# conroi/lcpc

Measured on AMD Instinct MI355X. Metric: field-elements committed/sec (whole node), Ligero 2^26 coeffs, higher is better.
Workload: dtype u32 limbs (255-bit prime field Ft255, Montgomery form)

## Files before the change

### lcpc_amd/csrc/ctx.cpp

```cpp
#include "internal.h"
#include <chrono>

using namespace lcpc;

namespace lcpc {


const uint8_t LBL_DT[7] = "$l//DT", LBL_PR[7] = "$l//PR", LBL_PE[7] = "$l//PE", LBL_CO[7] = "$l//CO";

void ctx_ref(lcpc_ctx* c) { c->refs.fetch_add(1); }

static void ctx_free(lcpc_ctx* c) {
  (void)hipSetDevice(c->prm.device);
  comm_release(c);
  for (const NttStep& s : c->ntt) dev_free(s.pack);
  dev_free(c->d_wq_w); dev_free(c->d_rootsls); dev_free(c->d_rootslcs);
  dev_free(c->d_rootsl); dev_free(c->d_rootslc); dev_free(c->d_qpl); dev_free(c->d_roots); dev_free(c->d_r2);
  dev_free(c->ws.d_tmp); dev_free(c->ws.d_t); dev_free(c->ws.d_mid); dev_free(c->d_scratch);
  c->verify_sets.clear();
  if (c->s_verify) (void)hipStreamDestroy(c->s_verify);
  for (unsigned k = 0; k < lcpc_ctx::N_STAGE; k++) {
    if (c->h_stage[k]) (void)hipHostFree(c->h_stage[k]);
    if (c->ev_stage[k]) (void)hipEventDestroy(c->ev_stage[k]);
  }
  for (auto* v : {&c->d_pre, &c->d_post})
    for (auto& d : *v) { dev_free(d.rowptr); dev_free(d.colidx); dev_free(d.vals); dev_free(d.vals29); }
  delete c;
}
void ctx_unref(lcpc_ctx* c) {
  if (c->refs.fetch_sub(1) == 1) ctx_free(c);
}

uint64_t ntt_mid_rows(const lcpc_ctx* c, uint64_t n_rows) {
  const bool ev = c->sw_ntt_mid_max_mb >= 0;
  if (c->ntt.size() != 2 || c->ntt[0].kernel != NttStep::K1S || n_rows == 0) return 0;
  if (!ev && c->log_n > 15) return 0;
  const uint64_t max_mb = ev ? (uint64_t)c->sw_ntt_mid_max_mb : 6144;
  if (max_mb == 0) return 0;
  const uint64_t per_row = c->n_cols * 36;
  uint64_t fit = (max_mb << 20) / per_row;
  if (fit == 0) return 0;
  if (fit >= n_rows) return n_rows;
  const uint64_t batches = (n_rows + fit - 1) / fit;
  return (n_rows + batches - 1) / batches;
}

static void wmul_table(const FieldDesc& f, const uint64_t* w_mont, int N, int W, uint32_t out[96]) {
  uint64_t v[MAXL];
  h_canon(f, v, w_mont);
  memset(out, 0, 96 * 4);
  for (int j = 0; j < N; j++) {
    uint64_t m[5] = {0, 0, 0, 0, 0};
    for (int i = 0; i < f.L; i++) m[i] = v[i];
    bool big = false;
    for (int i = f.L - 1; i >= 0; i--) {
      const uint64_t h = (f.p[i] >> 1) | (i + 1 < f.L ? f.p[i + 1] << 63 : 0);
      if (v[i] != h) { big = v[i] > h; break; }
    }
    if (big) {
      unsigned __int128 br = 0;
      for (int i = 0; i < 5; i++) { const unsigned __int128 d = (unsigned __int128)m[i] - (i < f.L ? f.p[i] : 0) - (uint64_t)br; m[i] = (uint64_t)d; br = (d >> 64) & 1; }
    }
    for (int k = 0; k < N; k++) {
      const int b = W * k, wd = b / 64, sh = b % 64;
      uint64_t x = m[wd] >> sh;
      if (sh && wd + 1 < 5) x |= m[wd + 1] << (64 - sh);
      out[N * k + j] = k < N - 1 ? (uint32_t)(x & (((uint64_t)1 << W) - 1)) : (uint32_t)x;
    }
    for (int s = 0; s < W; s++) h_add(f, v, v, v);
  }
}
static int build_wq_w(lcpc_ctx* c, int N, int W) {
  const FieldDesc* f = c->f;
  uint64_t i4[MAXL];
  memcpy(i4, f->rou, 8 * f->L);
  for (unsigned i = 0; i + 2 < f->S; i++) h_mul(*f, i4, i4, i4);
  uint32_t wt[96];
  wmul_table(*f, i4, N, W, wt);
  int rc = dev_alloc(&c->err, &c->d_wq_w, sizeof wt);
  if (rc) return rc;
  HIPCHK(c, hipMemcpy(c->d_wq_w, wt, sizeof wt, hipMemcpyHostToDevice));
  return 0;
}

static std::vector<uint32_t> clamp_table(const FieldDesc& f, int N, int W, int stride) {
  std::vector<uint32_t> tab((size_t)64 * stride, 0);
  for (int i = 0; i < 64; i++) {
    const int q = i - 24;
    uint64_t mag[5] = {0, 0, 0, 0, 0};
    unsigned __int128 cy = 0;
    for (int w = 0; w < 5; w++) { cy += (unsigned __int128)(w < f.L ? f.p[w] : 0) * (uint64_t)(q < 0 ? -q : q); mag[w] = (uint64_t)cy; cy >>= 64; }
    if (q < 0) {
      unsigned __int128 c2 = 1;
      for (int w = 0; w < 5; w++) { c2 += (unsigned __int128)(~mag[w]); mag[w] = (uint64_t)c2; c2 >>= 64; }
    }
    for (int l = 0; l < N; l++) {
      const int b = W * l, w = b / 64, sh = b % 64;
      uint64_t x = mag[w] >> sh;
      if (sh && w + 1 < 5) x |= mag[w + 1] << (64 - sh);
      tab[(size_t)i * stride + l] = l + 1 < N ? (uint32_t)(x & (((uint64_t)1 << W) - 1)) : (uint32_t)x;
    }
  }
  return tab;
}
static int limb_consts(lcpc_ctx* c, std::vector<uint32_t**>* made) {
  const int N = ntt_lns_limbs(c->NL), W = ntt_lns_limb_bits(c->NL);
  const std::vector<uint32_t> tab = clamp_table(*c->f, N, W, ntt_lns_stride(c->NL));
  if (made) { made->push_back(&c->d_qpl); made->push_back(&c->d_wq_w); }
  if (int rc = dev_alloc(&c->err, &c->d_qpl, tab.size() * 4)) return rc;
  HIPCHK(c, hipMemcpy(c->d_qpl, tab.data(), tab.size() * 4, hipMemcpyHostToDevice));
  return build_wq_w(c, N, W);
}

static void plan_passes(lcpc_ctx* c) {
  const unsigned k = c->log_n;
  const int NL = c->NL;
  const int lt_small = NL >= 6 ? 10 : (NL == 4 ? 11 : 12);
  const int lt_big = NL >= 6 ? 11 : 12;
  unsigned ltj_min = 0;
  while (((size_t)NL * 4 << ltj_min) < 128) ltj_min++;
  c->ntt.clear();
  auto add = [&](unsigned t0, unsigned s, unsigned log_tj, int lt) {
    NttStep p;
    p.log_tile = lt;
    p.a.roots = c->d_roots; p.a.roots29 = c->d_rootsl; p.a.qp29 = c->d_qpl; p.a.wq_w = c->d_wq_w;
    p.a.log_n = k; p.a.t0 = t0; p.a.s = s; p.a.log_tj = log_tj;
    p.roots29c = c->d_rootslc;
    p.mont_prefix = t0 + s == k ? (k == 0 ? 1u : (s % 2 == 0 ? 4u : 2u)) : 0u;
    c->ntt.push_back(p);
  };
  if ((int)k <= lt_small) {
    add(0, k, 0, lt_small);
    return;
  }
  int LT = lt_small;
  auto n_pass = [&](int lt) { unsigned per = lt - ltj_min, rest = k - lt; return 1 + (rest + per - 1) / per; };
  if (c->L == 4 && (k == 19 || k == 20) && !c->sw_ntt_general) {
    add(0, k - 10, 20 - k, 10);
    add(k - 10, 10, 0u, 10);
    return;
  }
  if (n_pass(lt_small) > 2 && n_pass(lt_big) < n_pass(lt_small)) LT = lt_big;
  const unsigned P = n_pass(LT);
  const unsigned s_final = LT;
  unsigned rem = k - s_final, t0 = 0;
  for (unsigned i = 0; i + 1 < P; i++) {
    const unsigned left = P - 1 - i;
    const unsigned s = (rem + left - 1) / left;
    add(t0, s, (uint32_t)LT - s, LT);
    t0 += s;
    rem -= s;
  }
  add(t0, s_final, 0u, LT);
}

static uint32_t ntt_tile_group_of(uint32_t log_n, int L, uint32_t log_tj) {
  const uint32_t tiles_log = log_n - 10;
  if (tiles_log < 3) return 0;
  uint32_t run_log = log_tj;
  for (uint32_t b = 8u * (uint32_t)L; b > 1; b >>= 1) run_log++;
  uint32_t lg = run_log <= 5 ? 11 - run_log : (run_log < 10 ? 10 - run_log : 0);
  return std::min(std::min(lg, 6u), tiles_log - 3);
}

static int build_limb_plan(lcpc_ctx* c, unsigned n_pass) {
  std::vector<uint32_t**> made;
  std::vector<NttStep> plan(n_pass);
  const int rc = [&]() -> int {
    const FieldDesc* f = c->f;
    ErrText* err = &c->err;
    const unsigned k = c->log_n, s0 = k - 10 * (n_pass - 1);
    const size_t stride = (size_t)ntt_lns_stride(c->NL);
    auto alloc = [&](uint32_t** p, size_t bytes) { made.push_back(p); return dev_alloc(err, p, bytes); };
    int r;
    if (c->L != 4) {
      uint64_t rp[2 * MAXL] = {1, 0, 0, 0};
      for (int i = 0; i < ntt_lns_limbs(c->NL) * ntt_lns_limb_bits(c->NL); i++) h_add(*f, rp, rp, rp);
      h_canon(*f, rp + f->L, rp);
      const size_t n_roots = (size_t)1 << (k - 1);
      uint32_t* d_rp = nullptr;
      if ((r = dev_alloc(err, &d_rp, 16 * f->L))) return r;
      if ((r = alloc(&c->d_rootsl, n_roots * stride * 4)) || (r = alloc(&c->d_rootslc, n_roots * stride * 4))) { dev_free(d_rp); return r; }
      hipError_t he = hipMemcpy(d_rp, rp, 16 * f->L, hipMemcpyHostToDevice);
      if (he == hipSuccess) he = launch_ntt_lns_roots(c->NL, c->d_roots, n_roots, d_rp, c->d_rootsl, nullptr);
      if (he == hipSuccess) he = launch_ntt_lns_roots(c->NL, c->d_roots, n_roots, d_rp + 2 * f->L, c->d_rootslc, nullptr);
      if (he == hipSuccess) he = hipDeviceSynchronize();
      dev_free(d_rp);
      if (he != hipSuccess) return fail_hip(err, he, "ntt_lns tables");
      if ((r = limb_consts(c, &made))) return r;
    }
    if (n_pass == 3) {
      const size_t n_sub = (size_t)1 << 19;
      if ((r = alloc(&c->d_rootsls, n_sub * stride * 4)) || (r = alloc(&c->d_rootslcs, n_sub * stride * 4))) return r;
      for (int i = 0; i < 2; i++) {
        const uint32_t* tab = i ? c->d_rootslc : c->d_rootsl;
        uint32_t* sub = i ? c->d_rootslcs : c->d_rootsls;
        HIPCHK(c, launch_ntt_lns_subtable(c->NL, tab, s0, n_sub, sub, nullptr));
      }
    }
    for (unsigned i = 0; i < n_pass; i++) {
      NttStep& p = plan[i];
      const bool sub = n_pass == 3 && i > 0, last = i + 1 == n_pass;
      p.kernel = c->L == 4 ? NttStep::K1S : NttStep::K1N;
      p.first = !last;
      p.a.roots = c->d_roots; p.a.roots29 = sub ? c->d_rootsls : c->d_rootsl; p.a.qp29 = c->d_qpl; p.a.wq_w = c->d_wq_w;
      p.a.log_n = sub ? 20u : k;
      p.a.t0 = last ? p.a.log_n - 10 : 0u;
      p.a.s = i == 0 ? s0 : 10u;
      p.a.log_tj = 10 - p.a.s;
      p.a.tile_group = p.first ? ntt_tile_group_of(p.a.log_n, c->L, p.a.log_tj) : 0u;
      p.a.canon_row_mask = sub ? (1u << (k - 20)) - 1 : 0u;
      p.roots29c = sub ? c->d_rootslcs : c->d_rootslc;
      p.mont_prefix = last && c->NL == 2 ? 4u : 0u;
      p.blk0_gone = last && c->NL != 2 && plan[i - 1].a.s >= 8 ? 1u : 0u;
      const bool nf = c->L == 4 && n_pass == 2 && (c->sw_ntt_form == 1 || (c->sw_ntt_form < 0 && s0 >= 6));
      p.a.form = nf ? 1u : 0u;
      if (nf && last) p.blk0_gone = 1u;
      p.pack_info = nf ? ntt_l9s_form_pack_info(p.a.s, p.first) : ntt_lns_pack_info(c->NL, p.a.s, p.first);
      const uint32_t n_classes = p.first != nf ? 1u << (p.a.log_n - 10) : 1u;
#ifdef LCPC_TEST_HOOKS
      if (n_pass == 3 && i == 0 && c->sw_test_fail_3pass) return LCPC_ERR_NOMEM;
#endif
      if ((r = alloc(&p.pack, (size_t)n_classes * p.pack_info.class_words * 4))) return r;
      NttPassArgs pa{};
      pa.roots29 = p.a.roots29; pa.roots29c = p.roots29c; pa.log_n = p.a.log_n; pa.t0 = p.a.t0; pa.s = p.a.s; pa.log_tj = p.a.log_tj;
      if (nf) HIPCHK(c, launch_ntt_l9s_form_pack(pa, p.first, p.pack_info, n_classes, p.pack, nullptr));
      else HIPCHK(c, launch_ntt_lns_pack(c->NL, pa, p.first, p.pack_info, n_classes, p.pack, nullptr));
    }
    HIPCHK(c, hipDeviceSynchronize());
    return 0;
  }();
  if (rc == 0) {
    c->ntt = std::move(plan);
    c->comm_canon = true;
    return 0;
  }
  for (uint32_t** p : made) { dev_free(*p); *p = nullptr; }
  if (rc != LCPC_ERR_NOMEM) return rc;
  (void)hipGetLastError();
  c->err.clear();
  return 0;
}

#define ECHK(call)                                                        \
  do {                                                                    \
    hipError_t e__ = (call);                                              \
    if (e__ != hipSuccess) return fail_hip(err, e__, #call);              \
  } while (0)

int encode_rows_device(const lcpc_ctx* c, EncodeWs* ws, const EncodeJob& j, hipStream_t st, ErrText* err, uint32_t* launches) {
  uint32_t dummy = 0;
  uint32_t& nl = launches ? *launches : dummy;
  if (j.kept_t) *j.kept_t = false;
  const uint64_t n_rows = j.n_rows;
  if (n_rows == 0) return 0;
  if (c->prm.encoding == LCPC_ENC_LIGERO) {
    uint64_t rb = ws->mid_failed ? 0 : ntt_mid_rows(c, n_rows);
    if (rb) {
      ErrText scratch_err;
      uint64_t want = rb * c->n_cols * 36;
#ifdef LCPC_TEST_HOOKS
      if (c->sw_test_fail_mid) want = (uint64_t)1 << 62;
#endif
      if (ensure_dev(&scratch_err, &ws->d_mid, &ws->mid_cap, want)) {
        (void)hipGetLastError();
        ws->mid_failed = true; ws->mid_cap = 0; rb = 0;
      }
    }
    const uint64_t batch = rb ? rb : n_rows;
    for (uint64_t r0 = 0; r0 < n_rows; r0 += batch) {
      const uint64_t nr = std::min(batch, n_rows - r0), consumed = r0 * j.src_stride;
      for (size_t i = 0; i < c->ntt.size(); i++) {
        const NttStep& p = c->ntt[i];
        const bool first = i == 0;
        const uint64_t len = (uint64_t)1 << p.a.log_n;
        NttPassArgs a = p.a;
        if (j.canon_out) { a.roots29c = p.roots29c; a.mont_prefix = p.mont_prefix; a.blk0_gone = p.blk0_gone; }
        a.dst = j.dst + r0 * c->n_cols * c->NL;
        a.src = first ? j.src + consumed * c->NL : a.dst;
        a.src_stride = first ? j.src_stride : len;
        a.dst_stride = len;
        a.n_valid = first ? j.n_valid : len;
        a.n_src_total = !first || j.n_src_total == ~(uint64_t)0 ? ~(uint64_t)0 : (j.n_src_total > consumed ? j.n_src_total - consumed : 0);
        a.copy_dst = first && j.copy_dst ? j.copy_dst + consumed * c->NL : nullptr;
        a.n_rows = nr << (c->log_n - p.a.log_n);
        a.mid = rb ? ws->d_mid : nullptr;
        switch (p.kernel) {
          case NttStep::K1S: ECHK(launch_ntt_pass_l9s(a, p.first, p.pack, p.pack_info, st)); break;
          case NttStep::K1N: ECHK(launch_ntt_pass_lns(c->NL, a, p.first, p.pack, p.pack_info, st)); break;
          case NttStep::GENERAL: ECHK(launch_ntt_pass(c->NL, p.log_tile, a, st)); break;
        }
        nl++;
      }
    }
    return 0;
  }
  const size_t t = c->d_pre.size();
  const DevCsr& pl = c->d_pre[t - 1];
  const size_t eb = elem_bytes(c);
  if (int rc = ensure_dev(err, &ws->d_tmp, &ws->tmp_cap, n_rows * pl.n_out * eb)) return rc;
  if (n_rows >= SDIG_T_MIN_ROWS) {
    if (int rc = ensure_dev(err, &ws->d_t, &ws->t_cap, n_rows * c->n_cols * eb)) return rc;
    ECHK(launch_transpose_to_t(c->NL, j.src, j.src_stride, j.n_valid, n_rows, ws->d_t, st, j.n_src_total, j.copy_dst, j.canon_out && j.keep_t));
    nl++;
    SpmmTArgs a{};
    a.t = ws->d_t; a.n_rows = n_rows;
    auto mat = [&](const DevCsr& m, uint64_t in_off, uint64_t out_off, bool to_tmp) -> int {
      a.out_alt = to_tmp ? ws->d_tmp : nullptr; a.in_off = in_off; a.out_off = out_off;
      a.rowptr = m.rowptr; a.colidx = m.colidx; a.vals = m.vals; a.vals29 = m.vals29; a.m = m.n_out;
      ECHK(launch_spmm_t(c->NL, a, st));
      nl++;
      return 0;
    };
    auto rs = [&](uint64_t out_off, uint64_t n_out) -> int {
      ECHK(launch_sdig_rs_t(c->NL, ws->d_tmp, (uint32_t)pl.n_out, ws->d_t, out_off, (uint32_t)n_out, n_rows, c->d_r2, st));
      nl++;
      return 0;
    };
    if (int rc = sdig_walk(c, mat, rs)) return rc;
    if (j.keep_t) {
      if (j.kept_t) *j.kept_t = true;
      return 0;
    }
    ECHK(launch_transpose_from_t(c->NL, ws->d_t, c->n_cols, n_rows, j.dst, c->n_cols, st));
    nl++;
    return 0;
  }
  if (j.src != j.dst || j.src_stride != c->n_cols) {
    ECHK(launch_pad_rows(c->NL, j.src, j.src_stride, j.dst, c->n_cols, j.n_valid, n_rows, st));
    nl++;
  }
  SpmvArgs a{};
  a.mat = j.dst; a.stride = c->n_cols; a.n_rows = n_rows;
  auto mat = [&](const DevCsr& m, uint64_t in_off, uint64_t out_off, bool to_tmp) -> int {
    a.out_alt = to_tmp ? ws->d_tmp : nullptr; a.in_off = in_off; a.out_off = out_off;
    if (to_tmp) a.out_alt_stride = pl.n_out;
    a.rowptr = m.rowptr; a.colidx = m.colidx; a.vals = m.vals; a.vals29 = m.vals29; a.m = m.n_out;
    ECHK(launch_spmv(c->NL, a, st));
    nl++;
    return 0;
  };
  auto rs = [&](uint64_t out_off, uint64_t n_out) -> int {
    ECHK(launch_sdig_rs(c->NL, ws->d_tmp, pl.n_out, (uint32_t)pl.n_out, j.dst, c->n_cols, out_off, (uint32_t)n_out, n_rows, c->d_r2, st));
    nl++;
    return 0;
  };
  return sdig_walk(c, mat, rs);
}

}

extern "C" {

int lcpc_abi_version(void) { return LCPC_ABI_VERSION; }

const char* lcpc_strerror(int s) {
  switch (s) {
    case LCPC_OK: return "ok";
    case LCPC_ERR_TOO_BIG: return "n_cols is too large for this encoding";
    case LCPC_ERR_ENCODE: return "encoding error";
    case LCPC_ERR_COMMIT: return "inconsistent commitment fields";
    case LCPC_ERR_COLUMN_NUMBER: return "bad column number";
    case LCPC_ERR_OUTER_TENSOR: return "outer tensor: wrong size";
    case LCPC_ERR_DIMS: return "dimensions not valid for this encoding";
    case LCPC_ERR_ARG: return "invalid argument";
    case LCPC_ERR_STATE: return "no commitment in this object";
    case LCPC_ERR_HIP: return "HIP runtime error";
    case LCPC_ERR_NOMEM: return "out of memory";
    case LCPC_ERR_NO_DEVICE: return "no usable HIP device (this library has no CPU fallback)";
    case LCPC_ERR_XCHG: return "all-gather of the sharded commit / prove failed";
    case LCPC_ERR_NO_RCCL: return "librccl could not be loaded";
    case LCPC_VERR_NUM_COL_OPENS: return "wrong number of column openings in proof";
    case LCPC_VERR_COLUMN_PATH: return "column verification: merkle path failed";
    case LCPC_VERR_COLUMN_EVAL: return "column verification: eval dot product failed";
    case LCPC_VERR_COLUMN_DEGREE: return "column verification: degree test dot product failed";
    case LCPC_VERR_OUTER_TENSOR: return "outer tensor: wrong size";
    case LCPC_VERR_INNER_TENSOR: return "inner tensor: wrong size";
    case LCPC_VERR_ENCODING_DIMS: return "encoding dimension mismatch";
    case LCPC_VERR_ENCODE: return "encoding error";
    case LCPC_VERR_MALFORMED: return "malformed proof bytes";
  }
  return "unknown status";
}
const char* lcpc_last_error(const lcpc_ctx* c) { return c ? c->err.c_str() : ""; }

int lcpc_static_get_dims(const lcpc_params* p, uint64_t* nr, uint64_t* np, uint64_t* nc) {
  if (!p || !nr || !np || !nc) return LCPC_ERR_ARG;
  LCPC_TRY
  const FieldDesc* f = field_desc((int)p->field);
  if (!f || p->n_coeffs == 0) return LCPC_ERR_ARG;
  if (p->encoding == LCPC_ENC_LIGERO) {
    if (p->rho_num == 0 || p->rho_num >= p->rho_den) return LCPC_ERR_ARG;
    return ligero_get_dims(*f, p->n_coeffs, p->rho_num, p->rho_den, nr, np, nc) ? LCPC_ERR_TOO_BIG : 0;
  } else if (p->encoding == LCPC_ENC_SDIG) {
    SdigSpec s;
    const int code = p->sdig_code ? (int)p->sdig_code : 3;
    uint64_t npr;
    if (!sdig_spec(code, &s) || !sdig_n_per_row(*f, p->n_coeffs, code, &npr)) return LCPC_ERR_ARG;
    std::vector<LevelDims> pre, post;
    if (!sdig_level_dims(s, npr, (double)f->flog2(), pre, post)) return LCPC_ERR_DIMS;
    *nr = (p->n_coeffs + npr - 1) / npr; *np = npr; *nc = sdig_codeword_length(pre, post);
    return 0;
  }
  return LCPC_ERR_ARG;
  LCPC_CATCH((lcpc_ctx*)nullptr)
}

int lcpc_static_get_dims_ml(const lcpc_params* p, uint32_t n_vars, uint64_t* nr, uint64_t* np, uint64_t* nc) {
  if (!p || !nr || !np || !nc || n_vars >= 63) return LCPC_ERR_ARG;
  LCPC_TRY
  const FieldDesc* f = field_desc((int)p->field);
  if (!f) return LCPC_ERR_ARG;
  const uint64_t n = (uint64_t)1 << n_vars;
  if (p->encoding == LCPC_ENC_LIGERO) {
    lcpc_params q = *p;
    q.n_coeffs = n;
    int rc = lcpc_static_get_dims(&q, nr, np, nc);
    if (rc) return rc;
    if ((*nr & (*nr - 1)) || (*np & (*np - 1)) || *nr * *np != n) return LCPC_ERR_DIMS;
    return 0;
  } else if (p->encoding == LCPC_ENC_SDIG) {
    SdigSpec s;
    const int code = p->sdig_code ? (int)p->sdig_code : 3;
    uint64_t npr;
    if (!sdig_spec(code, &s) || !sdig_n_per_row(*f, n, code, &npr, true)) return LCPC_ERR_ARG;
    std::vector<LevelDims> pre, post;
    if (!sdig_level_dims(s, npr, (double)f->flog2(), pre, post)) return LCPC_ERR_DIMS;
    *nr = (n + npr - 1) / npr; *np = npr; *nc = sdig_codeword_length(pre, post);
    return 0;
  }
  return LCPC_ERR_ARG;
  LCPC_CATCH((lcpc_ctx*)nullptr)
}

static int ctx_build(lcpc_ctx* c, const lcpc_params* p) {
  const FieldDesc* f = c->f;
  ErrText* err = &c->err;
  int rc = 0;
  if (p->encoding == LCPC_ENC_LIGERO) {
    if (p->rho_num == 0 || p->rho_num >= p->rho_den) return LCPC_ERR_ARG;
    uint64_t nr, np_, nc;
    if (p->n_per_row && p->n_cols) { np_ = p->n_per_row; nc = p->n_cols; }
    else if ((rc = lcpc_static_get_dims(p, &nr, &np_, &nc))) return rc;
    if (!(np_ < nc) || (nc & (nc - 1)) || log2_ceil(nc) > f->S) return LCPC_ERR_DIMS;
    if (log2_ceil(nc) > 30) return LCPC_ERR_TOO_BIG;
    c->n_per_row = np_; c->n_cols = nc; c->log_n = (unsigned)log2_ceil(nc);
    {
      const unsigned log_half = c->log_n ? c->log_n - 1 : 0;
      const size_t n_roots = (size_t)1 << log_half;
      std::vector<uint64_t> pw((size_t)(log_half + 1) * f->L);
      uint64_t w[MAXL];
      memcpy(w, f->rou, 8 * f->L);
      for (unsigned i = 0; i < f->S - c->log_n; i++) h_mul(*f, w, w, w);
      for (unsigned j = 0; j <= log_half; j++) { memcpy(&pw[(size_t)j * f->L], w, 8 * f->L); h_mul(*f, w, w, w); }
      uint32_t *d_pw = nullptr, *d_one = nullptr;
      if ((rc = dev_alloc(err, &d_pw, pw.size() * 8)) || (rc = dev_alloc(err, &d_one, 8 * f->L)) ||
          (rc = dev_alloc(err, &c->d_roots, n_roots * 8 * f->L)) ||
          (f->L == 4 && (rc = dev_alloc(err, &c->d_rootsl, n_roots * 48))) ||
          (f->L == 4 && (rc = dev_alloc(err, &c->d_rootslc, n_roots * 48)))) {
        dev_free(d_pw); dev_free(d_one);
        return rc;
      }
      hipError_t he = hipMemcpy(d_pw, pw.data(), pw.size() * 8, hipMemcpyHostToDevice);
      if (he == hipSuccess) he = hipMemcpy(d_one, f->r, 8 * f->L, hipMemcpyHostToDevice);
      if (he == hipSuccess) he = launch_roots(c->NL, d_pw, log_half, d_one, c->d_roots, c->d_rootsl, c->d_rootslc, nullptr);
      if (he == hipSuccess) he = hipDeviceSynchronize();
      dev_free(d_pw); dev_free(d_one);
      if (he != hipSuccess) return fail_hip(err, he, "precomp_fft");
    }
    if (f->L == 4) {
      if ((rc = limb_consts(c, nullptr))) return rc;
      c->comm_canon = true;
    }
    if ((rc = dev_alloc(err, &c->d_r2, 8 * f->L))) return rc;
    HIPCHK(c, hipMemcpy(c->d_r2, f->r2, 8 * f->L, hipMemcpyHostToDevice));
    plan_passes(c);
    if (c->sw_ntt_general) return 0;
    const uint32_t np = (uint32_t)c->ntt.size();
    if (c->L == 4 ? ntt_l9s_supported(c->log_n, np, c->ntt[0].log_tile) : np >= 2 && ntt_lns_supported(c->NL, c->log_n)) return build_limb_plan(c, 2);
    if (c->L == 4 ? ntt_l9s3_supported(c->log_n) : np >= 2 && ntt_lns3_supported(c->NL, c->log_n)) return build_limb_plan(c, 3);
    return 0;
  }
  if (p->encoding != LCPC_ENC_SDIG) return LCPC_ERR_ARG;
  if (!sdig_spec((int)c->prm.sdig_code, &c->spec)) return LCPC_ERR_ARG;
  uint64_t npr = p->n_per_row;
  if (!(p->n_per_row && p->n_cols)) {
    if (!sdig_n_per_row(*f, p->n_coeffs, (int)c->prm.sdig_code, &npr)) return LCPC_ERR_ARG;
  }
  std::vector<CsrMatrix> pre, post;
  const bool dbg = c->sw_debug_timing;
  auto now = [] { return std::chrono::duration<double, std::milli>(std::chrono::steady_clock::now().time_since_epoch()).count(); };
  const double t_gen0 = now();
  if (!sdig_generate(*f, c->spec, npr, p->seed, pre, post, c->pre_dims, c->post_dims)) return LCPC_ERR_DIMS;
  const double t_gen1 = now();
  c->n_per_row = npr;
  c->n_cols = sdig_codeword_length(c->pre_dims, c->post_dims);
  if (p->n_per_row && p->n_cols && p->n_cols != c->n_cols) return LCPC_ERR_DIMS;
  uint32_t* d_rprime = nullptr;
  if (f->L == 2 || f->L == 3) {
    uint64_t rp[MAXL] = {1, 0, 0, 0};
    for (int i = 0; i < ntt_lns_limbs(c->NL) * ntt_lns_limb_bits(c->NL); i++) h_add(*f, rp, rp, rp);
    if ((rc = dev_alloc(err, &d_rprime, 8 * f->L))) return rc;
    HIPCHK(c, hipMemcpy(d_rprime, rp, 8 * f->L, hipMemcpyHostToDevice));
  }
  struct FreeRp { uint32_t*& p; ~FreeRp() { if (p) { (void)hipDeviceSynchronize(); dev_free(p); p = nullptr; } } } free_rp{d_rprime};
  auto upload = [&](const CsrMatrix& m, DevCsr& d) -> int {
    d.n_in = m.n_in; d.n_out = m.n_out;
    int r;
    if ((r = dev_alloc(err, &d.rowptr, m.rowptr.size() * 4))) return r;
    if ((r = dev_alloc(err, &d.colidx, m.colidx.size() * 4))) return r;
    if ((r = dev_alloc(err, &d.vals, m.vals.size() * 8))) return r;
    HIPCHK(c, hipMemcpy(d.rowptr, m.rowptr.data(), m.rowptr.size() * 4, hipMemcpyHostToDevice));
    HIPCHK(c, hipMemcpy(d.colidx, m.colidx.data(), m.colidx.size() * 4, hipMemcpyHostToDevice));
    HIPCHK(c, hipMemcpy(d.vals, m.vals.data(), m.vals.size() * 8, hipMemcpyHostToDevice));
    if (f->L == 4) {
      const size_t nnz = m.colidx.size();
      if ((r = dev_alloc(err, &d.vals29, (nnz + 1) * 48))) return r;
      HIPCHK(c, launch_to_r29(d.vals, nnz, d.vals29, nullptr));
      HIPCHK(c, hipMemsetAsync(d.vals29 + nnz * 12, 0, 48, nullptr));
    } else if ((f->L == 2 || f->L == 3) && d_rprime) {
      const size_t nnz = m.colidx.size();
      const size_t stride = (size_t)ntt_lns_stride(c->NL);
      if ((r = dev_alloc(err, &d.vals29, (nnz + 1) * stride * 4))) return r;
      HIPCHK(c, launch_ntt_lns_roots(c->NL, d.vals, nnz, d_rprime, d.vals29, nullptr));
      HIPCHK(c, hipMemsetAsync(d.vals29 + nnz * stride, 0, stride * 4, nullptr));
    }
    return 0;
  };
  c->d_pre.resize(pre.size());
  c->d_post.resize(post.size());
  for (size_t i = 0; i < pre.size() && !rc; i++) { rc = upload(pre[i], c->d_pre[i]); if (!rc) rc = upload(post[i], c->d_post[i]); }
  if (!rc) rc = dev_alloc(err, &c->d_r2, 8 * f->L);
  if (rc) return rc;
  HIPCHK(c, hipMemcpy(c->d_r2, f->r2, 8 * f->L, hipMemcpyHostToDevice));
  if (dbg) fprintf(stderr, "[SdigEncoding::new] matgen %.1f ms, convert + upload %.1f ms\n", t_gen1 - t_gen0, now() - t_gen1);
  return 0;
}

int lcpc_ctx_create(const lcpc_params* p, lcpc_ctx** out) {
  if (!p || !out) return LCPC_ERR_ARG;
  *out = nullptr;
  lcpc_ctx* c = nullptr;
  LCPC_TRY
  const FieldDesc* f = field_desc((int)p->field);
  if (!f || p->hash > LCPC_HASH_SHA256) return LCPC_ERR_ARG;
  if (p->hash != LCPC_HASH_BLAKE3 && p->shard_count > 1) return LCPC_ERR_ARG;
  int ndev = 0;
  if (hipGetDeviceCount(&ndev) != hipSuccess || ndev <= 0 || p->device < 0 || p->device >= ndev) return LCPC_ERR_NO_DEVICE;
  if (hipSetDevice(p->device) != hipSuccess) return LCPC_ERR_NO_DEVICE;
  c = new lcpc_ctx();
  c->prm = *p;
  c->f = f; c->L = f->L; c->NL = 2 * f->L;
  if (c->prm.sdig_code == 0) c->prm.sdig_code = 3;
  c->sw_ntt_general = getenv("LCPC_NTT_GENERAL") != nullptr;
  if (const char* ev = getenv("LCPC_NTT_FORM")) c->sw_ntt_form = !strcmp(ev, "dif") ? 0 : (!strcmp(ev, "coset") ? 1 : -1);
  if (const char* ev = getenv("LCPC_NTT_MID_MAX_MB")) c->sw_ntt_mid_max_mb = (int64_t)strtoull(ev, nullptr, 10);
  if (const char* ev = getenv("LCPC_HOST_STAGE")) c->sw_host_stage = (int32_t)strtol(ev, nullptr, 10);
  c->sw_debug_timing = getenv("LCPC_DEBUG_TIMING") != nullptr;
#ifdef LCPC_TEST_HOOKS
  if (const char* ev = getenv("LCPC_TEST_FAIL")) {
    c->sw_test_fail_3pass = strstr(ev, "3pass") != nullptr;
    c->sw_test_fail_mid = strstr(ev, "mid") != nullptr;
  }
#endif
  int rc = 0;
  if (c->prm.shard_count > 1 && c->prm.shard_rank >= c->prm.shard_count) rc = LCPC_ERR_ARG;
  if (!rc) rc = ctx_build(c, p);
  if (rc) { ctx_unref(c); return rc; }
  c->np2 = next_pow2(c->n_cols);
  c->path_len = (uint32_t)log2_ceil(c->n_cols);
  if (c->sw_host_stage > 0) {
    c->stage_cap = (size_t)64 << 20;
    for (unsigned k = 0; k < 2; k++) {
      if (hipHostMalloc(reinterpret_cast<void**>(&c->h_stage[k]), c->stage_cap, hipHostMallocDefault) != hipSuccess) { (void)hipGetLastError(); c->h_stage[k] = nullptr; break; }
      if (hipEventCreateWithFlags(&c->ev_stage[k], hipEventDisableTiming) != hipSuccess) { (void)hipGetLastError(); (void)hipHostFree(c->h_stage[k]); c->h_stage[k] = nullptr; c->ev_stage[k] = nullptr; break; }
    }
  }
  *out = c;
  return 0;
  } catch (...) {
    if (c) ctx_unref(c);
    return LCPC_ERR_NOMEM;
  }
}

void lcpc_ctx_destroy(lcpc_ctx* c) {
  if (c) ctx_unref(c);
}

int lcpc_get_dims(const lcpc_ctx* c, uint64_t len, uint64_t* nr, uint64_t* np, uint64_t* nc) {
  if (!c || len == 0) return LCPC_ERR_ARG;
  if (nr) *nr = (len + c->n_per_row - 1) / c->n_per_row;
  if (np) *np = c->n_per_row;
  if (nc) *nc = c->n_cols;
  return 0;
}
int lcpc_dims_ok(const lcpc_ctx* c, uint64_t n_per_row, uint64_t n_cols) {
  if (!c) return 0;
  bool ok = n_per_row < n_cols && n_per_row == c->n_per_row && n_cols == c->n_cols;
  if (c->prm.encoding == LCPC_ENC_LIGERO) ok = ok && (n_cols & (n_cols - 1)) == 0;
  return ok ? 1 : 0;
}
uint64_t lcpc_get_n_col_opens(const lcpc_ctx* c) {
  if (!c) return 0;
  return c->prm.encoding == LCPC_ENC_LIGERO ? ligero_n_col_opens(c->prm.rho_num, c->prm.rho_den) : sdig_n_col_opens((int)c->prm.sdig_code);
}
uint64_t lcpc_get_n_degree_tests(const lcpc_ctx* c) { return c ? n_degree_tests(128, c->n_cols, c->f->flog2()) : 0; }
uint32_t lcpc_field_limbs(const lcpc_ctx* c) { return c ? (uint32_t)c->L : 0; }

int lcpc_encode_rows(lcpc_ctx* c, uint64_t* rows, uint64_t n_rows) {
  if (!c || !rows) return LCPC_ERR_ARG;
  if (n_rows == 0) return 0;
  LCPC_TRY
  std::lock_guard<std::mutex> g(c->mu);
  HIPCHK(c, hipSetDevice(c->prm.device));
  const size_t bytes = (size_t)n_rows * c->n_cols * elem_bytes(c);
  int rc = ensure_dev(&c->err, &c->d_scratch, &c->scratch_cap, bytes);
  if (rc) return rc;
  HIPCHK(c, hipMemcpy(c->d_scratch, rows, bytes, hipMemcpyHostToDevice));
  EncodeJob j;
  j.src = c->d_scratch; j.src_stride = c->n_cols; j.n_valid = c->n_cols; j.dst = c->d_scratch; j.n_rows = n_rows;
  if ((rc = encode_rows_device(c, &c->ws, j, nullptr, &c->err, nullptr))) return rc;
  HIPCHK(c, hipMemcpy(rows, c->d_scratch, bytes, hipMemcpyDeviceToHost));
  return 0;
  LCPC_CATCH(c)
}

}

namespace lcpc {
int encode_msgs_host(lcpc_ctx* c, const uint64_t* const* msgs, uint64_t n_rows, uint64_t* out) {
  if (n_rows == 0) return 0;
  std::lock_guard<std::mutex> g(c->mu);
  HIPCHK(c, hipSetDevice(c->prm.device));
  if (!c->s_verify) HIPCHK(c, hipStreamCreateWithFlags(&c->s_verify, hipStreamNonBlocking));
  hipStream_t st = c->s_verify;
  struct Drain { hipStream_t st; ~Drain() { (void)hipStreamSynchronize(st); } } drain{st};
  const size_t eb = elem_bytes(c);
  const size_t in_b = ((size_t)n_rows * c->n_per_row * eb + 255) & ~(size_t)255, out_b = (size_t)n_rows * c->n_cols * eb;
  int rc = ensure_dev(&c->err, &c->d_scratch, &c->scratch_cap, in_b + out_b);
  if (rc) return rc;
  uint8_t* base = reinterpret_cast<uint8_t*>(c->d_scratch);
  for (uint64_t i = 0; i < n_rows; i++)
    HIPCHK(c, hipMemcpyAsync(base + i * c->n_per_row * eb, msgs[i], c->n_per_row * eb, hipMemcpyHostToDevice, st));
  EncodeJob j;
  j.src = reinterpret_cast<uint32_t*>(base); j.src_stride = c->n_per_row; j.n_valid = c->n_per_row;
  j.dst = reinterpret_cast<uint32_t*>(base + in_b); j.n_rows = n_rows;
  if ((rc = encode_rows_device(c, &c->ws, j, st, &c->err, nullptr))) return rc;
  HIPCHK(c, hipMemcpyAsync(out, base + in_b, out_b, hipMemcpyDeviceToHost, st));
  HIPCHK(c, hipStreamSynchronize(st));
  return 0;
}
}

extern "C" {

int lcpc_field_sum_device(lcpc_ctx* c, const uint64_t* parts, uint32_t n_parts, uint64_t n_elems, void* stream, uint64_t* out) {
  if (!c || !parts || !out || n_parts == 0) return LCPC_ERR_ARG;
  hipError_t he = hipSetDevice(c->prm.device);
  if (he == hipSuccess)
    he = launch_field_sum(c->NL, reinterpret_cast<const uint32_t*>(parts), n_parts, n_elems, reinterpret_cast<uint32_t*>(out), (hipStream_t)stream);
  if (he != hipSuccess) {
    std::lock_guard<std::mutex> g(c->mu);
    return fail_hip(&c->err, he, "lcpc_field_sum_device");
  }
  return 0;
}

void lcpc_root_bincode(const uint8_t root[32], uint8_t out[40]) {
  const uint64_t l = 32;
  memcpy(out, &l, 8);
  memcpy(out + 8, root, 32);
}
void lcpc_free(void* p) { lcpc::proof_buf_free(p); }

}
```

### lcpc_amd/csrc/field_ln.h

```cpp
#pragma once
#include "field_dev.h"

namespace lcpc {

template <int NL, int W> constexpr u32 mod_limb(int k) {
  const int b = W * k, w = b / 32, sh = b % 32;
  const u64 lo = Mod<NL>::P[w], hi = (w + 1 < NL) ? Mod<NL>::P[w + 1] : 0;
  return (u32)(((lo | (hi << 32)) >> sh) & ((1u << W) - 1));
}
template <int FID> struct LnField;
template <> struct LnField<FT63> {
  static constexpr int FID = FT63, N = 3, W = 26, NL = 2, WAVES = 8, STRIDE = 4;
  static constexpr u32 limb(int k) { return mod_limb<NL, W>(k); }
};
template <> struct LnField<FT127> {
  static constexpr int FID = FT127, N = 5, W = 29, NL = 4, WAVES = 7, STRIDE = 8;
  static constexpr u32 limb(int k) { return mod_limb<NL, W>(k); }
};
template <> struct LnField<FT191> {
  static constexpr int FID = FT191, N = 7, W = 29, NL = 6, WAVES = 5, STRIDE = 8;
  static constexpr u32 limb(int k) { return mod_limb<NL, W>(k); }
};
template <> struct LnField<FT255> {
  static constexpr int FID = FT255, N = 9, W = 29, NL = 8, WAVES = 4, STRIDE = 12;
  static constexpr u32 limb(int k) { return mod_limb<NL, W>(k); }
};

#include "field_ln_gen.h"
#include "field_r29_gen.h"
#include "field_wmul_gen.h"

template <int N> struct LN {
  u32 v[N];
};

namespace ln {
constexpr int QOFF = 24;
constexpr int QBIAS = 40;

template <class FT> LCPC_DEV LN<FT::N> from_packed(const Fe<FT::NL>& a) {
  constexpr int N = FT::N, W = FT::W, NL = FT::NL;
  LN<N> r;
#pragma unroll
  for (int k = 0; k < N; k++) {
    const int b = W * k, w = b / 32, sh = b % 32;
    u32 x;
    if (sh == 0) x = a.v[w];
    else if (w + 1 < NL) x = __builtin_amdgcn_alignbit(a.v[w + 1], a.v[w], sh);
    else x = a.v[w] >> sh;
    r.v[k] = k + 1 < N ? (x & ((1u << W) - 1)) : x;
  }
  return r;
}
template <class FT> LCPC_DEV void to_packed(u32* out, const u32* l) {
  constexpr int N = FT::N, W = FT::W, NL = FT::NL;
#pragma unroll
  for (int w = 0; w < NL; w++) {
    u32 x = 0;
#pragma unroll
    for (int k = 0; k < N; k++) {
      const int off = W * k - 32 * w;
      if (off >= 0 && off < 32) x |= l[k] << off;
      else if (off < 0 && off > -32) x |= l[k] >> (-off);
    }
    out[w] = x;
  }
}
template <int N> LCPC_DEV LN<N> load_limbs(const u32* t) {
  LN<N> r;
  if constexpr (N == 3) {
    const uint2 a = *reinterpret_cast<const uint2*>(t);
    r.v[0] = a.x; r.v[1] = a.y; r.v[2] = t[2];
  } else {
    const uint4 a = *reinterpret_cast<const uint4*>(t);
    r.v[0] = a.x; r.v[1] = a.y; r.v[2] = a.z; r.v[3] = a.w;
    if constexpr (N == 5) r.v[4] = t[4];
    else if constexpr (N == 7) { const uint2 b = *reinterpret_cast<const uint2*>(t + 4); r.v[4] = b.x; r.v[5] = b.y; r.v[6] = t[6]; }
    else { const uint4 b = *reinterpret_cast<const uint4*>(t + 4); r.v[4] = b.x; r.v[5] = b.y; r.v[6] = b.z; r.v[7] = b.w; r.v[8] = t[8]; }
  }
  return r;
}
template <int N> LCPC_DEV LN<N> add(const LN<N>& a, const LN<N>& b) {
  LN<N> r;
#pragma unroll
  for (int k = 0; k < N; k++) r.v[k] = a.v[k] + b.v[k];
  return r;
}
template <int N> LCPC_DEV LN<N> sub(const LN<N>& a, const LN<N>& b) {
  LN<N> r;
#pragma unroll
  for (int k = 0; k < N; k++) r.v[k] = a.v[k] - b.v[k];
  return r;
}
template <class FT> LCPC_DEV void normalize(LN<FT::N>& a) {
#pragma unroll
  for (int k = 0; k + 1 < FT::N; k++) {
    a.v[k + 1] += (u32)((int32_t)a.v[k] >> FT::W);
    a.v[k] &= (1u << FT::W) - 1;
  }
}
template <class FT> LCPC_DEV u32 clamp_q(u32 top) {
  constexpr u32 PTOP1 = FT::limb(FT::N - 1) + 1;
  constexpr int SH = 31 - __builtin_clz(PTOP1);
  constexpr u32 MAGIC = (u32)((((u64)1 << (32 + SH)) + PTOP1 - 1) / PTOP1);
  static_assert((u64)64 * PTOP1 * PTOP1 < ((u64)1 << (32 + SH)), "magic division range");
  const u32 n = top + (u32)(QOFF * PTOP1 - QBIAS);
  return __umulhi(n, MAGIC) >> SH;
}
template <class FT> LCPC_DEV LN<FT::N> clamp_row(const u32* nqp, u32 q) { return load_limbs<FT::N>(nqp + q * FT::STRIDE); }
template <class FT> LCPC_DEV void clamp_apply(LN<FT::N>& a, const LN<FT::N>& nt) {
  int32_t c = 0;
#pragma unroll
  for (int k = 0; k + 1 < FT::N; k++) {
    const int32_t d = (int32_t)(a.v[k] + nt.v[k] + (u32)c);
    a.v[k] = (u32)d & ((1u << FT::W) - 1);
    c = d >> FT::W;
  }
  a.v[FT::N - 1] = a.v[FT::N - 1] + nt.v[FT::N - 1] + (u32)c;
}
template <class FT> LCPC_DEV LN<FT::N> mul(const LN<FT::N>& a, const LN<FT::N>& w) {
  LN<FT::N> r;
  if constexpr (FT::FID == FT63) ln_mul1s_ft63(a.v, w.v, r.v);
  else if constexpr (FT::FID == FT127) ln_mul1s_ft127(a.v, w.v, r.v);
  else if constexpr (FT::FID == FT191) ln_mul1s_ft191(a.v, w.v, r.v);
  else r29_mul1s(a.v, w.v, r.v);
  return r;
}
template <class FT> constexpr bool has_mul_u = FT::N >= 5;
template <class FT> LCPC_DEV LN<FT::N> mul_u(const LN<FT::N>& a, const u32* wt) {
  static_assert(has_mul_u<FT>, "no shifted-multiples multiply for this field");
  LN<FT::N> r;
  if constexpr (FT::FID == FT127) wmul_u_ft127(a.v, wt, r.v);
  else if constexpr (FT::FID == FT191) wmul_u_ft191(a.v, wt, r.v);
  else {
    u32 np2[9];
#pragma unroll
    for (int j = 0; j < 9; j++) np2[j] = 0u - 2u * FT::limb(j);
    wmul_u(a.v, np2, wt, r.v);
  }
  return r;
}
template <class FT> struct LazyN {
  u64 c[2 * FT::N];
};
template <class FT> LCPC_DEV void lazy_zero(LazyN<FT>& a) {
#pragma unroll
  for (int k = 0; k < 2 * FT::N; k++) a.c[k] = 0;
}
template <class FT> LCPC_DEV void lazy_mac(LazyN<FT>& a, const LN<FT::N>& x, const LN<FT::N>& v) {
#pragma unroll
  for (int i = 0; i < FT::N; i++)
#pragma unroll
    for (int j = 0; j < FT::N; j++) a.c[i + j] += (u64)x.v[i] * v.v[j];
}
template <class FT> LCPC_DEV void lazy_normalize(LazyN<FT>& a) {
#pragma unroll
  for (int k = 0; k + 1 < 2 * FT::N; k++) {
    a.c[k + 1] += a.c[k] >> FT::W;
    a.c[k] &= (1u << FT::W) - 1;
  }
}
template <class FT> LCPC_DEV Fe<FT::NL> lazy_reduce(LazyN<FT>& a) {
  constexpr int N = FT::N, W = FT::W;
  constexpr u32 M = (1u << W) - 1;
  lazy_normalize<FT>(a);
  u32 m[N], r[N];
  u64 acc = 0;
#pragma unroll
  for (int k = 0; k < 2 * N; k++) {
    acc += a.c[k];
#pragma unroll
    for (int i = 0; i < N; i++) {
      const int j = k - i;
      if (i < k && j >= 1 && j < N) acc += (u64)m[i] * FT::limb(j);
    }
    if (k < N) {
      m[k] = (0u - (u32)acc) & M;
      acc += m[k];
      acc >>= W;
    } else {
      r[k - N] = (u32)acc & M;
      acc >>= W;
    }
  }
  u32 t[FT::NL];
  to_packed<FT>(t, r);
  return fe_reduce_once<FT::NL>(t);
}

LCPC_DEV void clamp(LN<9>& a, const u32* qp) {
  constexpr u32 M = (1u << 29) - 1;
  constexpr u32 PTOP1 = LnField<FT255>::limb(8) + 1;
  constexpr u64 MAGIC = (((u64)1 << 52) + PTOP1 - 1) / PTOP1;
  const u32 n = a.v[8] + (u32)(QOFF * PTOP1 - QBIAS);
  const u32 q = (u32)(((u64)n * MAGIC) >> 52);
  const u32* t = qp + q * 12;
  int32_t d[9];
#pragma unroll
  for (int k = 0; k < 9; k++) d[k] = (int32_t)(a.v[k] - t[k]);
#pragma unroll
  for (int k = 0; k < 8; k++) {
    d[k + 1] += d[k] >> 31;
    a.v[k] = (u32)d[k] & M;
  }
  a.v[8] = (u32)d[8];
}
LCPC_DEV Fe<8> to_packed_reduced(LN<9> a, const u32* qp) {
  clamp(a, qp);
  u32 t[8];
  to_packed<LnField<FT255>>(t, a.v);
  return fe_reduce_once<8>(t);
}
}

LCPC_DEV Fe<8> fe_mul_r29(const Fe<8>& a, const LN<9>& b) {
  const LN<9> x = ln::from_packed<LnField<FT255>>(a);
  u32 m[9], r[9];
  r29_columns(x.v, b.v, m, r);
  u32 t[8];
  ln::to_packed<LnField<FT255>>(t, r);
  return fe_reduce_once<8>(t);
}

LCPC_DEV Fe<8> fe_canon_r29(const Fe<8>& a) {
  using FT = LnField<FT255>;
  constexpr u32 M = (1u << 29) - 1;
  u32 x[9];
#pragma unroll
  for (int k = 0; k < 9; k++) {
    const int b = 29 * k - 5;
    u32 v;
    if (k == 0) v = (a.v[0] << 5);
    else {
      const int w = b / 32, sh = b % 32;
      if (sh == 0) v = a.v[w];
      else if (w + 1 < 8) v = __builtin_amdgcn_alignbit(a.v[w + 1], a.v[w], sh);
      else v = a.v[w] >> sh;
    }
    x[k] = v & M;
  }
  u32 m[9], r[9];
  u64 acc = 0;
#pragma unroll
  for (int k = 0; k < 17; k++) {
    if (k < 9) acc += x[k];
#pragma unroll
    for (int i = 0; i < 9; i++) {
      const int j = k - i;
      if (i < k && j >= 1 && j < 9) acc += (u64)m[i] * FT::limb(j);
    }
    if (k < 9) {
      m[k] = (0u - (u32)acc) & M;
      acc += m[k];
      acc >>= 29;
    } else {
      r[k - 9] = (u32)acc & M;
      acc >>= 29;
    }
  }
  r[8] = (u32)acc;
  u32 t[8];
  ln::to_packed<FT>(t, r);
  return fe_reduce_once<8>(t);
}

}
```

### lcpc_amd/csrc/gen/gen_r29_asm.py

```python
#!/usr/bin/env python3

N = 9


def block(terms, a_name, b_name):
    ins = []
    ops = []
    idx = {}

    def op(name, k):
        key = (name, k)
        if key not in idx:
            idx[key] = len(ops) + 1
            ops.append('"v"(%s[%d])' % (name, k) if name != "P" else '"s"(LnField<FT255>::limb(%d))' % k)
        return "%%%d" % idx[key]

    for i, j in terms:
        ins.append('"v_mad_u64_u32 %%0, vcc, %s, %s, %%0\\n\\t"' % (op(a_name, i), op(b_name, j)))
    return "    asm(" + "\n        ".join(ins) + '\n        : "+v"(acc) : ' + ", ".join(ops) + ' : "vcc");'


out = []
out.append("// GENERATED by lcpc_amd/csrc/gen/gen_r29_asm.py -- do not edit.  Column chains of fe_mul_r29 (see field_ln.h).")
out.append("// x: multiplicand limbs (u32[9]), b: twiddle limbs (u32[9]), m: quotient digits, r: result limbs")
out.append("LCPC_DEV void r29_columns(const u32* x, const u32* b, u32* m, u32* r) {")
out.append("  u64 acc = 0;")
for k in range(2 * N - 1):
    prod = [(i, k - i) for i in range(N) if 0 <= k - i < N]
    red = [(i, k - i) for i in range(N) if i < k and 1 <= k - i < N]
    out.append("  {  // column %d: %d products, %d reduction terms" % (k, len(prod), len(red)))
    out.append(block(prod, "x", "b"))
    if red:
        out.append(block(red, "m", "P"))
    if k < N:
        out.append("    m[%d] = (0u - (u32)acc) & 0x1fffffffu;" % k)
        out.append('    asm("v_mad_u64_u32 %%0, vcc, %%1, 1, %%0" : "+v"(acc) : "v"(m[%d]) : "vcc");   // + m_k * p_0 (= 1)' % k)
        out.append("    acc >>= 29;")
    else:
        out.append("    r[%d] = (u32)acc & 0x1fffffffu;" % (k - N))
        out.append("    acc >>= 29;")
    out.append("  }")
out.append("  r[8] = (u32)acc;")
out.append("}")


FT255_P = 0x663c799b6e4d2900fda9df04b9575969ef73c79086595f3002a4f20000000001
ACC = 126
PS = 92
acc = "v[%d:%d]" % (ACC, ACC + 1)
lo = "v%d" % ACC
R = lambda k: "%%%d" % k
X = lambda i: "%%%d" % (N + i)
B = lambda j: "%%%d" % (2 * N + j)
def mul1(signed):
    mad = "v_mad_i64_i32" if signed else "v_mad_u64_u32"
    shr = "v_ashrrev_i64" if signed else "v_lshrrev_b64"
    ins = []
    for j in range(1, N):
        pj = (FT255_P >> (29 * j)) & ((1 << 29) - 1)
        ins.append("s_mov_b32 s%d, 0x%x" % (PS + j - 1, ((-pj) & 0xffffffff) if signed else pj))
    first = True
    for k in range(2 * N - 1):
        for i in range(N):
            j = k - i
            if 0 <= j < N:
                ins.append("%s %s, vcc, %s, %s, %s" % (mad, acc, X(i), B(j), "0" if first else acc))
                first = False
        for i in range(N):
            j = k - i
            if i < k and 1 <= j < N:
                ins.append("%s %s, vcc, %s, s%d, %s" % (mad, acc, R(i), PS + j - 1, acc))
        if k < N and signed:
            ins.append("v_and_b32 %s, 0x1fffffff, %s" % (R(k), lo))
        elif k < N:
            ins.append("v_sub_u32 %s, 0, %s" % (R(k), lo))
            ins.append("v_and_b32 %s, 0x1fffffff, %s" % (R(k), R(k)))
            ins.append("v_mad_u64_u32 %s, vcc, %s, 1, %s" % (acc, R(k), acc))
        else:
            ins.append("v_and_b32 %s, 0x1fffffff, %s" % (R(k - N), lo))
        ins.append("%s %s, 29, %s" % (shr, acc, acc))
    ins.append("v_mov_b32 %s, %s" % (R(N - 1), lo))
    return ins


def emit(name, comment, ins):
    out.append("")
    out.append(comment)
    out.append("LCPC_DEV void %s(const u32* x, const u32* b, u32* r) {" % name)
    out.append("  asm(")
    for t in ins:
        out.append('      "%s\\n\\t"' % t)
    outs = ", ".join('"=&v"(r[%d])' % k for k in range(N))
    inps = ", ".join(['"v"(x[%d])' % i for i in range(N)] + ['"v"(b[%d])' % j for j in range(N)])
    clob = ", ".join(['"vcc"', '"v%d"' % ACC, '"v%d"' % (ACC + 1)] + ['"s%d"' % (PS + j) for j in range(N - 1)])
    out.append("      : %s\n      : %s\n      : %s);" % (outs, inps, clob))
    out.append("}")


out.append("")
out.append("// One-statement multiplies; they clobber v[%d:%d], s[%d:%d], vcc.  The asserts tie the literals to LnField<FT255>." % (ACC, ACC + 1, PS, PS + N - 2))
for j in range(1, N):
    out.append("static_assert(LnField<FT255>::limb(%d) == 0x%xu, \"gen_r29_asm.py modulus\");" % (j, (FT255_P >> (29 * j)) & ((1 << 29) - 1)))
emit("r29_mul1s", "// signed form (ln::mul<LnField<FT255>>): x limbs two's complement, |x_k| < 2^30, |value| < 16p; b as above.\n"
     "// r = x * b * 2^-261 in (-1.2p, 0.2p]: limbs 0..7 in [0, 2^29), top limb signed.", mul1(True))
print("\n".join(out))
```

### lcpc_amd/csrc/internal.h

```cpp
#pragma once
#include "../../include/lcpc_hip.h"
#include <hip/hip_runtime.h>
#include <stdio.h>
#include <stdlib.h>
#include <string.h>
#include <algorithm>
#include <atomic>
#include <condition_variable>
#include <memory>
#include <mutex>
#include <new>
#include <shared_mutex>
#include <string>
#include <thread>
#include <vector>
#include "encoding.h"
#include "host_crypto.h"
#include "host_field.h"
#include "host_par.h"
#include "kernels.h"

namespace lcpc {

struct DevCsr {
  uint64_t n_in = 0, n_out = 0;
  uint32_t *rowptr = nullptr, *colidx = nullptr, *vals = nullptr;
  uint32_t* vals29 = nullptr;
};
struct NttStep {
  enum Kernel { GENERAL, K1S, K1N } kernel = GENERAL;
  bool first = false;
  int log_tile = 0;
  NttPassArgs a{};
  const uint32_t* roots29c = nullptr;
  uint32_t mont_prefix = 0, blk0_gone = 0;
  uint32_t* pack = nullptr;
  NttPackInfo pack_info{};
};

struct EncodeWs {
  uint32_t* d_tmp = nullptr;
  uint64_t tmp_cap = 0;
  uint32_t* d_t = nullptr;
  uint64_t t_cap = 0;
  uint32_t* d_mid = nullptr;
  uint64_t mid_cap = 0;
  bool mid_failed = false;
};
uint64_t ntt_mid_rows(const lcpc_ctx* c, uint64_t n_rows);

constexpr uint64_t SDIG_T_MIN_ROWS = 24;

void* proof_buf_alloc(size_t n);
void proof_buf_free(void* p);

class ErrText {
 public:
  ErrText& operator=(const std::string& s) { set(s.c_str()); return *this; }
  ErrText& operator=(const char* s) { set(s); return *this; }
  void clear() { set(""); }
  const char* c_str() const { return buf_[cur_.load(std::memory_order_acquire)]; }
 private:
  void set(const char* s) {
    std::lock_guard<std::mutex> g(mu_);
    const unsigned k = (cur_.load(std::memory_order_relaxed) + 1) % 4;
    snprintf(buf_[k], sizeof buf_[k], "%s", s ? s : "");
    cur_.store(k, std::memory_order_release);
  }
  std::mutex mu_;
  std::atomic<unsigned> cur_{0};
  char buf_[4][512] = {};
};

class FillLock {
 public:
  void lock() {
    std::unique_lock<std::mutex> g(mu_);
    ++fills_waiting_;
    cv_.wait(g, [&] { return !filling_ && readers_ == 0; });
    --fills_waiting_;
    filling_ = true;
  }
  void unlock() {
    { std::lock_guard<std::mutex> g(mu_); filling_ = false; }
    cv_.notify_all();
  }
  void lock_shared() {
    std::unique_lock<std::mutex> g(mu_);
    cv_.wait(g, [&] { return !filling_ && fills_waiting_ == 0; });
    ++readers_;
  }
  void unlock_shared() {
    bool last;
    { std::lock_guard<std::mutex> g(mu_); last = --readers_ == 0; }
    if (last) cv_.notify_all();
  }
 private:
  std::mutex mu_;
  std::condition_variable cv_;
  unsigned readers_ = 0, fills_waiting_ = 0;
  bool filling_ = false;
};

struct DevScratch {
  uint32_t* d = nullptr;
  uint64_t cap = 0;
  uint32_t* t29 = nullptr;
  uint64_t t29_cap = 0;
  void release() { if (d) (void)hipFree(d); if (t29) (void)hipFree(t29); d = t29 = nullptr; cap = t29_cap = 0; }
};

struct CallSet {
  bool busy = false;
  uint8_t* h_pin = nullptr;
  uint64_t h_pin_cap = 0;
  hipStream_t st = nullptr;
  hipEvent_t ev_slice[2] = {nullptr, nullptr};
  DevScratch sc;
  int make();
  void quiesce() { (void)hipStreamSynchronize(st); }
  ~CallSet();
};
struct VerifySet {
  bool busy = false;
  uint8_t* h_pin = nullptr;
  uint64_t h_pin_cap = 0;
  int make() { return 0; }
  void quiesce() {}
  ~VerifySet() { if (h_pin) (void)hipHostFree(h_pin); }
};

template <typename S> class SetPool {
 public:
  static constexpr size_t MAX_SETS = 8;
  int take(uint64_t pin_bytes, S** out) {
    *out = nullptr;
    std::unique_lock<std::mutex> lk(mu_);
    bool reuse_only = false;
    for (;;) {
      S* pick = nullptr;
      for (auto& s : sets_) if (!s->busy && s->h_pin_cap >= pin_bytes) { pick = s.get(); break; }
      if (!pick && !reuse_only) {
        for (auto& s : sets_) if (!s->busy) { pick = s.get(); break; }
        if (!pick && sets_.size() < MAX_SETS) {
          std::unique_ptr<S> s(new S());
          if (int rc = s->make()) return rc;
          sets_.push_back(std::move(s));
          pick = sets_.back().get();
        }
      }
      if (!pick) {
        if (reuse_only && !any_holds(pin_bytes)) return LCPC_ERR_NOMEM;
        cv_.wait(lk);
        continue;
      }
      pick->busy = true;
      if (pick->h_pin_cap >= pin_bytes) { *out = pick; return 0; }
      lk.unlock();
      if (pick->h_pin) (void)hipHostFree(pick->h_pin);
      pick->h_pin = nullptr; pick->h_pin_cap = 0;
      void* hp = nullptr;
      const bool ok = hipHostMalloc(&hp, (size_t)pin_bytes, hipHostMallocDefault) == hipSuccess;
      if (!ok) (void)hipGetLastError();
      lk.lock();
      if (ok) { pick->h_pin = static_cast<uint8_t*>(hp); pick->h_pin_cap = pin_bytes; *out = pick; return 0; }
      pick->busy = false;
      if (!any_holds(pin_bytes)) return LCPC_ERR_NOMEM;
      reuse_only = true;
    }
  }
  void give(S* s) {
    { std::lock_guard<std::mutex> g(mu_); s->busy = false; }
    cv_.notify_all();
  }
  void clear() { sets_.clear(); }
 private:
  bool any_holds(uint64_t pin_bytes) const {
    for (auto& s : sets_) if (s->h_pin_cap >= pin_bytes) return true;
    return false;
  }
  std::mutex mu_;
  std::condition_variable cv_;
  std::vector<std::unique_ptr<S>> sets_;
};
template <typename S> struct SetLease {
  SetPool<S>& pool;
  S* s = nullptr;
  ~SetLease() { if (s) { s->quiesce(); pool.give(s); } }
};

struct BatchSlab {
  uint8_t* d = nullptr;
  uint64_t off_comm = 0, off_t = 0, off_coeffs = 0, off_hashes = 0, off_cvs = 0;
  uint64_t comm_stride = 0, t_stride = 0, coeffs_stride = 0, hashes_stride = 0, cvs_stride = 0;
  uint64_t tmp_stride = 0;
  uint32_t n_batch = 0;
  uint64_t n_rows = 0;
  uint32_t* h_roots = nullptr;
  uint32_t* d_roots_alias = nullptr;
  EncodeWs ws;
  uint32_t* seg(uint64_t off, uint64_t stride, uint32_t i) const { return reinterpret_cast<uint32_t*>(d + off) + (size_t)i * stride; }
  ~BatchSlab() {
    if (d) (void)hipFree(d);
    if (ws.d_tmp) (void)hipFree(ws.d_tmp);
    if (ws.d_t) (void)hipFree(ws.d_t);
    if (ws.d_mid) (void)hipFree(ws.d_mid);
    if (h_roots) (void)hipHostFree(h_roots);
  }
};

}

struct lcpc_transcript {
  lcpc::Transcript t;
  lcpc_transcript(const uint8_t* l, size_t n) : t(l, n) {}
};

struct lcpc_ctx {
  lcpc_params prm{};
  bool sw_ntt_general = false;
  int sw_ntt_form = -1;
  int64_t sw_ntt_mid_max_mb = -1;
  bool sw_debug_timing = false;
  bool sw_test_fail_3pass = false;
  bool sw_test_fail_mid = false;
  const lcpc::FieldDesc* f = nullptr;
  int L = 0, NL = 0;
  uint64_t n_per_row = 0, n_cols = 0, np2 = 0;
  uint32_t path_len = 0;
  unsigned log_n = 0;
  uint32_t* d_roots = nullptr;
  uint32_t* d_rootsl = nullptr;
  uint32_t* d_rootslc = nullptr;
  uint32_t* d_qpl = nullptr;
  uint32_t* d_rootsls = nullptr;
  uint32_t* d_rootslcs = nullptr;
  uint32_t* d_wq_w = nullptr;
  std::vector<lcpc::NttStep> ntt;
  bool comm_canon = false;
  lcpc::SdigSpec spec{};
  std::vector<lcpc::LevelDims> pre_dims, post_dims;
  std::vector<lcpc::DevCsr> d_pre, d_post;
  uint32_t* d_r2 = nullptr;
  lcpc::EncodeWs ws;
  uint32_t* d_scratch = nullptr;
  uint64_t scratch_cap = 0;
  void* comm = nullptr;
  std::mutex xchg_mu;
  hipEvent_t ev_xchg = nullptr;
  std::atomic<int> refs{1};
  lcpc::ErrText err;
  std::mutex mu;
  lcpc::SetPool<lcpc::VerifySet> verify_sets;
  hipStream_t s_verify = nullptr;
  std::mutex stage_mu;
  static constexpr unsigned N_STAGE = 4;
  uint8_t* h_stage[N_STAGE] = {nullptr, nullptr, nullptr, nullptr};
  hipEvent_t ev_stage[N_STAGE] = {nullptr, nullptr, nullptr, nullptr};
  size_t stage_cap = 0;
  unsigned stage_next = 0;
  int32_t sw_host_stage = -1;
};

struct lcpc_commit_s {
  lcpc_ctx* enc = nullptr;
  bool committed = false;
  uint64_t n_rows = 0;
  uint64_t row_begin = 0, n_rows_local = 0;
  uint64_t chunk_begin = 0, chunk_end = 0, n_chunks = 0;
  uint32_t *d_coeffs = nullptr, *d_comm = nullptr, *d_hashes = nullptr, *d_cvs = nullptr;
  const uint32_t* coeffs_view = nullptr;
  uint64_t cap_coeff_rows = 0, cap_comm_rows = 0, cap_cvs = 0;
  std::shared_ptr<lcpc::BatchSlab> slab;
  uint32_t slab_index = 0;
  uint32_t* d_chain = nullptr;
  uint64_t cap_chain = 0;
  lcpc::EncodeWs ws;
  bool comm_t = false;
  bool comm_rows_valid = false;
  uint32_t* d_node_tab = nullptr;
  uint64_t node_tab_key = 0;
  std::vector<uint32_t> node_slot_h, node_log_h;
  struct NodeTab { uint64_t key; uint32_t* d; std::vector<uint32_t> slot, lg; };
  std::vector<NodeTab> node_tabs;
  uint8_t* d_gather = nullptr;
  uint64_t gather_cap = 0;
  uint8_t *d_xsend = nullptr, *d_xrecv = nullptr;
  uint64_t xchg_cap = 0;
  lcpc::DevScratch sc;
  uint32_t* h_root = nullptr;
  uint32_t* d_root_alias = nullptr;
  bool timing = false;
  hipEvent_t ev[6] = {nullptr, nullptr, nullptr, nullptr, nullptr, nullptr};
  hipStream_t s_prove = nullptr;
  hipEvent_t ev_done = nullptr;
  hipStream_t s_xchg = nullptr;
  hipEvent_t ev_hashed = nullptr;
  bool shard_encoded = false;
  hipStream_t s_copy = nullptr, s_comp = nullptr;
  hipEvent_t ev_batch[16] = {nullptr};
  mutable lcpc::FillLock fill_mu;
  lcpc::SetPool<lcpc::CallSet> sets;
  std::mutex shard_prove_mu;
  lcpc_timings last{};
  uint32_t launches[3] = {0, 0, 0};
  lcpc::ErrText err;
  std::mutex mu;
};

namespace lcpc {

inline int fail_hip(ErrText* err, hipError_t e, const char* what) {
  if (err) *err = std::string(what) + ": " + hipGetErrorString(e);
  return e == hipErrorOutOfMemory ? LCPC_ERR_NOMEM : LCPC_ERR_HIP;
}
#define HIPCHK(c, call)                                                   \
  do {                                                                    \
    hipError_t e__ = (call);                                              \
    if (e__ != hipSuccess) return lcpc::fail_hip((c) ? &(c)->err : nullptr, e__, #call); \
  } while (0)

#define LCPC_TRY try {
#define LCPC_CATCH(c)                                                     \
  } catch (const std::bad_alloc&) {                                       \
    if (c) (c)->err = "host allocation failed";                          \
    return LCPC_ERR_NOMEM;                                                \
  } catch (const std::exception& ex__) {                                  \
    if (c) (c)->err = ex__.what();                                       \
    return LCPC_ERR_STATE;                                                \
  } catch (...) {                                                         \
    return LCPC_ERR_STATE;                                                \
  }

template <typename T> int dev_alloc(ErrText* err, T** p, size_t bytes) {
  *p = nullptr;
  if (bytes == 0) bytes = 16;
  hipError_t e = hipMalloc(reinterpret_cast<void**>(p), bytes);
  if (e != hipSuccess) return fail_hip(err, e, "hipMalloc");
  return 0;
}
inline void dev_free(void* p) { if (p) (void)hipFree(p); }
template <typename T> int ensure_dev(ErrText* err, T** p, uint64_t* cap, uint64_t bytes) {
  bytes = (bytes + 255) & ~(uint64_t)255;
  if (bytes > *cap || !*p) {
    dev_free(*p);
    *p = nullptr; *cap = 0;
    int rc = dev_alloc(err, p, (size_t)bytes);
    if (rc) return rc;
    *cap = bytes;
  }
  return 0;
}

inline size_t elem_bytes(const lcpc_ctx* c) { return (size_t)8 * c->L; }
inline bool is_sha3(const lcpc_ctx* c) { return c->prm.hash == LCPC_HASH_SHA3_256; }
inline bool is_blake2b(const lcpc_ctx* c) { return c->prm.hash == LCPC_HASH_BLAKE2B; }
inline bool is_keccak256(const lcpc_ctx* c) { return c->prm.hash == LCPC_HASH_KECCAK256; }
inline bool is_sha256(const lcpc_ctx* c) { return c->prm.hash == LCPC_HASH_SHA256; }
inline bool is_blake3(const lcpc_ctx* c) { return c->prm.hash == LCPC_HASH_BLAKE3; }
inline uint32_t digest_len(const lcpc_ctx* c) { return is_blake2b(c) ? 64u : 32u; }
inline uint32_t digest_words(const lcpc_ctx* c) { return digest_len(c) / 4; }
inline uint64_t leaf_chunks(const lcpc_ctx* c, uint64_t n_rows) { return (32 + elem_bytes(c) * n_rows + 1023) / 1024; }

extern const uint8_t LBL_DT[7], LBL_PR[7], LBL_PE[7], LBL_CO[7];


void ctx_ref(lcpc_ctx* c);
void ctx_unref(lcpc_ctx* c);
struct EncodeJob {
  const uint32_t* src = nullptr;
  uint64_t src_stride = 0, n_valid = 0;
  uint32_t* dst = nullptr;
  uint64_t n_rows = 0;
  uint64_t n_src_total = ~(uint64_t)0;
  uint32_t* copy_dst = nullptr;
  bool canon_out = false;
  bool keep_t = false;
  bool* kept_t = nullptr;
};
int encode_rows_device(const lcpc_ctx* c, EncodeWs* ws, const EncodeJob& j, hipStream_t st, ErrText* err, uint32_t* launches);

int encode_msgs_host(lcpc_ctx* c, const uint64_t* const* msgs, uint64_t n_rows, uint64_t* out);

template <class Mat, class Rs> int sdig_walk(const lcpc_ctx* c, Mat&& mat, Rs&& rs) {
  const size_t t = c->d_pre.size();
  const DevCsr& pl = c->d_pre[t - 1];
  uint64_t in_start = 0;
  for (size_t i = 0; i + 1 < t; i++) {
    if (int rc = mat(c->d_pre[i], in_start, in_start + c->d_pre[i].n_in, false)) return rc;
    in_start += c->d_pre[i].n_in;
  }
  if (int rc = mat(pl, in_start, 0, true)) return rc;
  const uint64_t in_end = in_start + pl.n_in;
  if (int rc = rs(in_end, c->d_post[t - 1].n_in)) return rc;
  in_start = in_end + pl.n_out;
  uint64_t out_start = in_end + c->d_post[t - 1].n_in;
  for (size_t ii = t; ii-- > 0;) {
    in_start -= c->d_pre[ii].n_out;
    if (int rc = mat(c->d_post[ii], in_start, out_start, false)) return rc;
    out_start += c->d_post[ii].n_out;
  }
  return 0;
}

int ensure_scratch(lcpc_commit_t* m, DevScratch* sc, uint64_t bytes);
int ensure_cvs(lcpc_commit_t* m, uint64_t n_chunks);
int begin_commit(lcpc_commit_t* m, hipStream_t st, uint64_t n_rows_total, uint64_t row_begin, uint64_t row_end, uint64_t chunk_begin,
                 uint64_t chunk_end);
int ensure_commit_buffers(lcpc_commit_t* m, uint64_t n_rows_local, bool own_coeffs, bool comm_rows);
void leave_slab(lcpc_commit_t* m);
int ensure_comm_rows(lcpc_commit_t* m);
int merkleize_device(lcpc_commit_t* m, hipStream_t st);
int commit_device_locked(lcpc_commit_t* m, const uint64_t* coeffs_dev, uint64_t n_coeffs, hipStream_t st, uint32_t flags, uint8_t* root);
int encode_coeffs(lcpc_commit_t* m, const uint32_t* src, uint64_t n_src, bool borrow, hipStream_t st);
int hash_chunks(lcpc_commit_t* m, uint64_t a, uint64_t b, uint32_t* out, hipStream_t st);
int merkle_top(lcpc_commit_t* m, hipStream_t st, uint32_t levels_done = 0);
int seal_commit(lcpc_commit_t* m, hipStream_t st, uint8_t* root);
int order_after_commit(lcpc_commit_t* m, hipStream_t st);
int collapse_run(lcpc_commit_t* m, DevScratch* sc, const uint32_t* d_tensors, uint32_t n_tensors, hipStream_t st, uint32_t* d_polys);
size_t collapse_scratch_bytes(const lcpc_commit_t* m, uint32_t n_tensors);
int take_call_set(lcpc_commit_t* m, uint64_t pin_bytes, CallSet** ws);
int collapse_host(lcpc_commit_t* m, CallSet* ws, const uint64_t* tensors, uint32_t n_tensors, uint64_t* polys, uint64_t* polys_canon);
int collapse_host_sliced(lcpc_commit_t* m, CallSet* ws, const uint64_t* tensor, uint64_t* polys, uint64_t* polys_canon, uint64_t* cut_out);
int collapse_wait_slice(lcpc_commit_t* m, CallSet* ws, int s);
int open_columns_host(lcpc_commit_t* m, CallSet* ws, const uint64_t* cols, uint32_t n, uint64_t* col_vals, size_t vals_pitch, uint8_t* paths);
int open_columns_device(lcpc_commit_t* m, const uint64_t* d_cols, uint32_t n, uint32_t* d_vals, uint32_t* d_paths, hipStream_t st);

void shard_layout_of(const lcpc_ctx* c, uint64_t g, uint64_t n_rows, uint64_t* rb, uint64_t* re, uint64_t* cb, uint64_t* ce, uint64_t* nch);
int shard_nodes(uint64_t c0, uint64_t c1, uint64_t* first, uint32_t* lg);
void shard_chunk_range(uint64_t F, uint64_t n_chunks, uint64_t G, uint64_t g, uint64_t* c0, uint64_t* c1);
void comm_release(lcpc_ctx* c);
struct ShardXchg {
  uint8_t *send_dev, *recv_dev;
  uint64_t max_bytes;
  lcpc_allgather_fn fn;
  void* user;
  bool stream_ordered = false;
};
int prove_stream(lcpc_commit_t* m, hipStream_t* st);
int collapse_sharded(lcpc_commit_t* m, const ShardXchg& x, const uint64_t* tensors_full, uint32_t nt, uint64_t* polys, uint64_t* polys_canon);
int open_sharded(lcpc_commit_t* m, const ShardXchg& x, const uint64_t* cols, uint32_t n, uint64_t* vals, size_t vals_pitch, uint8_t* paths);

int prove_impl(lcpc_commit_t* m, const uint64_t* outer, uint64_t n_outer, lcpc_transcript* trw, uint8_t** proof, uint64_t* proof_len,
               uint64_t* cols_opened, const ShardXchg* xchg);

}
```

### lcpc_amd/csrc/kernels.h

```cpp
#pragma once
#include <hip/hip_runtime.h>
#include <stdint.h>

namespace lcpc {

struct NttPassArgs {
  const uint32_t* src;
  uint32_t* dst;
  const uint32_t* roots;
  const uint32_t* roots29;
  const uint32_t* qp29;
  const uint32_t* roots29c;
  uint32_t mont_prefix;
  uint64_t src_stride, dst_stride;
  uint64_t n_valid;
  uint64_t n_src_total;
  uint32_t* copy_dst;
  uint64_t n_rows;
  uint32_t log_n, t0, s, log_tj;
  uint32_t* mid = nullptr;
  uint32_t canon_row_mask = 0;
  uint32_t blk0_gone = 0;
  const uint32_t* wq_w = nullptr;
  uint32_t tile_group = 0;
  uint32_t form = 0;
};
hipError_t launch_ntt_pass(int nl, int log_tile, const NttPassArgs& a, hipStream_t st);

struct NttPackInfo {
  uint32_t round_off[8];
  uint32_t class_words;
  uint32_t u_off;
};
bool ntt_l9s_supported(uint32_t log_n, uint32_t n_passes, int log_tile);
bool ntt_l9s3_supported(uint32_t log_n);
hipError_t launch_ntt_pass_l9s(const NttPassArgs& a, bool first, const uint32_t* pack, const NttPackInfo& pi, hipStream_t st);
NttPackInfo ntt_l9s_form_pack_info(uint32_t s, bool first);
hipError_t launch_ntt_l9s_form_pack(const NttPassArgs& a, bool first, const NttPackInfo& pi, uint32_t n_classes, uint32_t* pack, hipStream_t st);

bool ntt_lns_supported(int nl, uint32_t log_n);
bool ntt_lns3_supported(int nl, uint32_t log_n);
hipError_t launch_ntt_pass_lns(int nl, const NttPassArgs& a, bool first, const uint32_t* pack, const NttPackInfo& pi, hipStream_t st);
int ntt_lns_limbs(int nl);
int ntt_lns_limb_bits(int nl);
int ntt_lns_stride(int nl);
hipError_t launch_ntt_lns_subtable(int nl, const uint32_t* tab, uint32_t shift, uint64_t n, uint32_t* sub, hipStream_t st);
NttPackInfo ntt_lns_pack_info(int nl, uint32_t s, bool first);
hipError_t launch_ntt_lns_roots(int nl, const uint32_t* roots, uint64_t n, const uint32_t* rprime, uint32_t* out, hipStream_t st);
hipError_t launch_ntt_lns_pack(int nl, const NttPassArgs& a, bool first, const NttPackInfo& pi, uint32_t n_classes, uint32_t* pack, hipStream_t st);

hipError_t launch_roots(int nl, const uint32_t* pw, uint32_t log_half, const uint32_t* one, uint32_t* roots, uint32_t* roots29,
                        uint32_t* roots29c, hipStream_t st);

struct LeafArgs {
  const uint32_t* comm;
  uint64_t row_stride;
  uint64_t col_stride;
  uint64_t n_cols;
  int64_t  row_base;
  uint64_t n_rows_total;
  uint32_t chunk_begin, n_chunks_local, n_chunks_total;
  uint32_t* out;
  uint32_t canon_in;
};
hipError_t launch_leaf_chunks(int nl, const LeafArgs& a, hipStream_t st);
hipError_t launch_leaf_finish(uint32_t* cvs, uint32_t n_chunks, uint64_t n_cols, uint32_t* digests, hipStream_t st);
hipError_t launch_leaf_finish_nodes(uint32_t* cvs, const uint32_t* node_slot, const uint32_t* node_log, uint32_t n_nodes,
                                    uint64_t n_cols, uint32_t* out, bool root, hipStream_t st);
hipError_t launch_merkle_tree(uint32_t* hashes, uint64_t np2, hipStream_t st, uint32_t* root_out);
hipError_t launch_merkle_tree_from(uint32_t* hashes, uint64_t np2, uint32_t levels_done, hipStream_t st, uint32_t* root_out);
bool leaf_tree_supported(const LeafArgs& a, uint64_t np2);
hipError_t launch_leaf_tree(int nl, const LeafArgs& a, uint32_t* hashes, uint64_t np2, hipStream_t st);

hipError_t launch_leaf_chunks_batch(int nl, const LeafArgs& a, uint32_t n_batch, uint64_t comm_stride, uint64_t out_stride, hipStream_t st);
hipError_t launch_leaf_finish_batch(uint32_t* cvs, uint32_t n_chunks, uint64_t n_cols, uint32_t* digests, uint32_t n_batch, uint64_t cvs_stride,
                                    uint64_t digests_stride, hipStream_t st);
hipError_t launch_leaf_tree_batch(int nl, const LeafArgs& a, uint32_t* hashes, uint64_t np2, uint32_t n_batch, uint64_t comm_stride,
                                  uint64_t hashes_stride, hipStream_t st);
hipError_t launch_merkle_tree_from_batch(uint32_t* hashes, uint64_t np2, uint32_t levels_done, uint32_t n_batch, uint64_t hashes_stride,
                                         hipStream_t st, uint32_t* root_out);
hipError_t launch_batch_place(const uint64_t* src, uint64_t src_stride, uint64_t n_valid, uint64_t* dst, uint64_t dst_stride, uint32_t n_batch,
                              hipStream_t st);

hipError_t launch_sha3_leaves_batch(int nl, const LeafArgs& a, uint32_t n_batch, uint64_t comm_stride, uint64_t out_stride, hipStream_t st);
hipError_t launch_keccak256_leaves_batch(int nl, const LeafArgs& a, uint32_t n_batch, uint64_t comm_stride, uint64_t out_stride, hipStream_t st);
hipError_t launch_sha256_leaves_batch(int nl, const LeafArgs& a, uint32_t n_batch, uint64_t comm_stride, uint64_t out_stride, hipStream_t st);
hipError_t launch_blake2b_leaves_batch(int nl, const LeafArgs& a, uint32_t n_batch, uint64_t comm_stride, uint64_t out_stride, hipStream_t st);
hipError_t launch_sha3_merkle_tree_batch(uint32_t* hashes, uint64_t np2, uint32_t n_batch, uint64_t hashes_stride, hipStream_t st, uint32_t* root_out);
hipError_t launch_keccak256_merkle_tree_batch(uint32_t* hashes, uint64_t np2, uint32_t n_batch, uint64_t hashes_stride, hipStream_t st,
                                              uint32_t* root_out);
hipError_t launch_sha256_merkle_tree_batch(uint32_t* hashes, uint64_t np2, uint32_t n_batch, uint64_t hashes_stride, hipStream_t st,
                                           uint32_t* root_out);
hipError_t launch_blake2b_merkle_tree_batch(uint32_t* hashes, uint64_t np2, uint32_t n_batch, uint64_t hashes_stride, hipStream_t st,
                                            uint32_t* root_out);

hipError_t launch_sha3_leaves(int nl, const LeafArgs& a, hipStream_t st);
hipError_t launch_sha3_merkle_tree(uint32_t* hashes, uint64_t np2, hipStream_t st, uint32_t* root_out);
hipError_t launch_keccak256_leaves(int nl, const LeafArgs& a, hipStream_t st);
hipError_t launch_keccak256_merkle_tree(uint32_t* hashes, uint64_t np2, hipStream_t st, uint32_t* root_out);

hipError_t launch_sha256_leaves(int nl, const LeafArgs& a, hipStream_t st);
hipError_t launch_sha256_merkle_tree(uint32_t* hashes, uint64_t np2, hipStream_t st, uint32_t* root_out);

hipError_t launch_blake2b_leaves(int nl, const LeafArgs& a, hipStream_t st);
hipError_t launch_blake2b_merkle_tree(uint32_t* hashes, uint64_t np2, hipStream_t st, uint32_t* root_out);
hipError_t launch_blake2b_gather_paths(const uint32_t* hashes, uint64_t np2, uint32_t path_len, const uint64_t* cols, uint32_t n,
                                       uint32_t* paths, hipStream_t st);

inline uint64_t sha3_leaf_blocks(int nl, uint64_t n_rows_total) { return (4 + (uint64_t)(nl / 2) * n_rows_total) / 17 + 1; }
inline uint64_t sha256_leaf_blocks(int nl, uint64_t n_rows_total) {
  const uint64_t w = 4 + (uint64_t)(nl / 2) * n_rows_total;
  return w / 8 + 1 + ((w & 7) == 7 ? 1 : 0);
}
inline uint64_t blake2b_leaf_blocks(int nl, uint64_t n_rows_total) { return (8 + (uint64_t)(nl / 2) * n_rows_total + 15) / 16; }
constexpr uint32_t SHA3_STATE_WORDS = 50, SHA256_STATE_WORDS = 8, BLAKE2B_STATE_WORDS = 16;
hipError_t launch_sha3_leaves_range(int nl, const LeafArgs& a, uint64_t blk_begin, uint64_t blk_end, uint64_t* state, hipStream_t st);
hipError_t launch_keccak256_leaves_range(int nl, const LeafArgs& a, uint64_t blk_begin, uint64_t blk_end, uint64_t* state, hipStream_t st);
hipError_t launch_sha256_leaves_range(int nl, const LeafArgs& a, uint64_t blk_begin, uint64_t blk_end, uint32_t* state, hipStream_t st);
hipError_t launch_blake2b_leaves_range(int nl, const LeafArgs& a, uint64_t blk_begin, uint64_t blk_end, uint64_t* state, hipStream_t st);

struct CollapseArgs {
  const uint32_t* coeffs;
  const uint32_t* tensors;
  const uint32_t* tensors29;
  uint32_t* out;
  uint64_t n_rows, n_per_row;
  uint32_t n_tensors, n_splits;
  uint64_t j0 = 0, j1 = 0, out_stride = 0;
};
hipError_t launch_collapse(int nl, const CollapseArgs& a, hipStream_t st);
hipError_t launch_to_r29(const uint32_t* in, uint64_t n, uint32_t* out, hipStream_t st);
hipError_t launch_field_sum(int nl, const uint32_t* parts, uint32_t n_parts, uint64_t n_elems, uint32_t* out, hipStream_t st);

hipError_t launch_gather_columns(int nl, const uint32_t* comm, uint64_t n_rows, uint64_t row_stride, uint64_t col_stride,
                                 const uint64_t* cols, uint32_t n, uint32_t* vals, const uint32_t* r2, hipStream_t st);
hipError_t launch_to_mont(int nl, const uint32_t* in, uint64_t n, const uint32_t* r2, uint32_t* out, hipStream_t st);
hipError_t launch_to_canon(int nl, const uint32_t* in, uint64_t n, uint32_t* out, hipStream_t st);
hipError_t launch_assemble_columns(int nl, const uint32_t* recv, uint64_t block_words, const uint64_t* rb, uint32_t G, uint32_t n,
                                   uint64_t n_rows, uint32_t* out, hipStream_t st);
hipError_t launch_gather_paths(const uint32_t* hashes, uint64_t np2, uint32_t path_len, const uint64_t* cols, uint32_t n,
                               uint32_t* paths, hipStream_t st);

struct SpmvArgs {
  uint32_t* mat;
  uint32_t* out_alt;
  uint64_t stride, out_alt_stride;
  uint64_t in_off, out_off;
  const uint32_t* rowptr;
  const uint32_t* colidx;
  const uint32_t* vals;
  const uint32_t* vals29;
  uint64_t m, n_rows;
};
hipError_t launch_spmv(int nl, const SpmvArgs& a, hipStream_t st);
hipError_t launch_transpose_to_t(int nl, const uint32_t* src, uint64_t src_stride, uint64_t n_valid, uint64_t n_rows,
                                 uint32_t* t, hipStream_t st, uint64_t n_src_total = ~(uint64_t)0, uint32_t* copy_dst = nullptr,
                                 bool canon = false);
hipError_t launch_transpose_from_t(int nl, const uint32_t* t, uint64_t n_pos, uint64_t n_rows, uint32_t* dst,
                                   uint64_t dst_stride, hipStream_t st);
struct SpmmTArgs {
  uint32_t* t;
  uint32_t* out_alt;
  uint64_t n_rows;
  uint64_t in_off, out_off;
  const uint32_t* rowptr;
  const uint32_t* colidx;
  const uint32_t* vals;
  const uint32_t* vals29;
  uint64_t m;
};
hipError_t launch_spmm_t(int nl, const SpmmTArgs& a, hipStream_t st);
hipError_t launch_sdig_rs_t(int nl, const uint32_t* in_t, uint32_t n_in, uint32_t* t, uint64_t out_off, uint32_t n_out,
                            uint64_t n_rows, const uint32_t* r2, hipStream_t st);
hipError_t launch_transpose_to_t_batch(int nl, const uint32_t* src, uint64_t src_stride, uint64_t n_valid, uint64_t n_rows, uint32_t* t,
                                       uint32_t n_batch, uint64_t t_stride, hipStream_t st, uint64_t n_src_total = ~(uint64_t)0,
                                       uint32_t* copy_dst = nullptr, bool canon = false);
hipError_t launch_spmm_t_batch(int nl, const SpmmTArgs& a, uint32_t n_batch, uint64_t t_stride, uint64_t out_alt_stride, hipStream_t st);
hipError_t launch_sdig_rs_t_batch(int nl, const uint32_t* in_t, uint32_t n_in, uint32_t* t, uint64_t out_off, uint32_t n_out,
                                  uint64_t n_rows, const uint32_t* r2, uint32_t n_batch, uint64_t in_stride, uint64_t t_stride,
                                  hipStream_t st);

hipError_t launch_sdig_rs(int nl, const uint32_t* in, uint64_t in_stride, uint32_t n_in, uint32_t* mat, uint64_t stride,
                          uint64_t out_off, uint32_t n_out, uint64_t n_rows, const uint32_t* r2, hipStream_t st);
hipError_t launch_pad_rows(int nl, const uint32_t* src, uint64_t src_stride, uint32_t* dst, uint64_t dst_stride,
                           uint64_t n_valid, uint64_t n_rows, hipStream_t st);

}
```

### lcpc_amd/csrc/ntt_l9s.hip

```cpp
#include "kernels.h"
#include "ntt_ln_dev.h"

namespace lcpc {

namespace {

template <int S, int LTJ, bool FIRST, bool MID, bool NF>
__global__ void __launch_bounds__(256, 4) ntt_pass_l9s_kernel(NttPassArgs a, const u32* __restrict__ pack, NttPackInfo pi) {
  using FT = LnField<FT255>;
  constexpr int NL = 8, LT = S + LTJ, LBT = LTJ;
  constexpr bool LAST = !FIRST;
  static_assert(LT == 10, "1024-element tiles: one radix-4 quad (two radix-2 pairs) per thread and round");
  static_assert(FIRST || (LTJ == 0 && S % 2 == 0), "the last pass works on contiguous tiles and ends with the trivial stages k-2, k-1");
  using SH = Shape<S, LBT>;
  using SP = PureShape<S>;
  constexpr int RU = NF ? (FIRST ? SP::RU : -1) : SH::RU;
  constexpr int RC = NF && FIRST ? SP::RC : -1;
  constexpr bool SWZD = NF ? (LAST || SP::RU >= 0) : RU >= 0;
  auto SWZ = [](u32 e) -> u32 {
    if constexpr (NF && LAST) return e ^ (((e >> 4) & 3u) * 5u);
    else if constexpr (NF && FIRST && SWZD && LBT == 2) return e ^ ((((e >> 4) ^ (e >> 6)) & 3u) << 2);
    else if constexpr (SWZD) return e ^ ((e >> 4) & 15u);
    else return e;
  };
  extern __shared__ __attribute__((aligned(16))) u32 lds[];
  constexpr u32 T = 1u << LT;
  u32* nqp = lds + (size_t)T * 9;
  const u32 k = a.log_n;
  const u32 tiles_per_row = 1u << (k - LT);
  u64 row;
  u32 tile;
  if (FIRST && a.tile_group) {
    const u32 lg = a.tile_group;
    const u32 xcd = blockIdx.x & 7u;
    const u64 qq = blockIdx.x >> 3;
    const u32 sub = (u32)qq & ((1u << lg) - 1);
    const u64 q2 = qq >> lg;
    tile = (((u32)(q2 / a.n_rows) * 8u + xcd) << lg) | sub;
    row = q2 % a.n_rows;
  } else if (tiles_per_row >= 8) {
    const u32 xcd = blockIdx.x & 7u;
    const u64 qq = blockIdx.x >> 3;
    tile = (u32)(qq / a.n_rows) * 8u + xcd;
    row = qq % a.n_rows;
  } else {
    row = blockIdx.x / tiles_per_row;
    tile = blockIdx.x % tiles_per_row;
  }
  const u32 tid = threadIdx.x;
  mem_phase(true);
  const u32 lb = FIRST ? k - S : 0u;
  auto gindex = [&](u32 e) -> u32 {
    if constexpr (FIRST) return ((e >> LBT) << lb) | (tile << LTJ) | (e & ((1u << LBT) - 1));
    else return (tile << S) | e;
  };
  const bool canon = a.roots29c != nullptr && ((u32)row & a.canon_row_mask) == 0;
  for (u32 i = tid; i < 64 * 12; i += 256) nqp[i] = 0u - a.qp29[i];
  const u32* src = a.src + row * a.src_stride * NL;
  constexpr bool DIRECT = !(LAST && MID);
  LN<9> xin[4];
  if constexpr (LAST && MID) {
    const uint4* t4 = reinterpret_cast<const uint4*>(a.mid + (row << k) * 9 + (size_t)tile * (9 * T));
    uint4* l4 = reinterpret_cast<uint4*>(lds);
    if constexpr (SWZD) {
#pragma unroll
      for (u32 i = tid; i < 2 * T; i += 256) l4[(i & ~(T - 1)) | SWZ(i & (T - 1))] = t4[i];
#pragma unroll
      for (u32 i = tid; i < T / 4; i += 256) {
        const uint4 v = t4[2 * T + i];
        const u32 b = 8 * T + SWZ(4 * i);
        lds[b] = v.x; lds[b ^ 1u] = v.y; lds[b ^ 2u] = v.z; lds[b ^ 3u] = v.w;
      }
    } else {
#pragma unroll
    for (u32 i = tid; i < 9 * T / 4; i += 256) l4[i] = t4[i];
    }
  } else {
#pragma unroll
  for (u32 it = 0; it < 4; it++) {
    const u32 e = tid + 256u * it;
    const u32 g = gindex(e);
    Fe<NL> v;
    if constexpr (FIRST) {
      v = (g < a.n_valid && row * a.src_stride + g < a.n_src_total) ? fe_load<NL>(src + (size_t)g * NL) : fe_zero<NL>();
      if (a.copy_dst != nullptr && g < a.n_valid) fe_store<NL>(a.copy_dst + (row * a.src_stride + g) * NL, v);
    } else {
      v = fe_load<NL>(src + (size_t)g * NL);
    }
    xin[it] = ln::from_packed<FT>(v);
  }
  __builtin_amdgcn_sched_barrier(0);
  }
  const u32* cls_pack = pack + (size_t)(FIRST != NF ? tile : 0u) * pi.class_words;
  const bool blk0_tile = (FIRST || tile == 0) && a.blk0_gone == 0;
  LN<9> k32;
#pragma unroll
  for (int i = 0; i < 9; i++) k32.v[i] = i == 0 ? 32u : 0u;
  const bool zero_hi = FIRST && a.n_valid <= (1ull << (k - 1));
  if constexpr (!DIRECT) __syncthreads();

  if constexpr (SH::U0 == 1) {
    constexpr u32 half = 1u << (S - 1 + LBT);
    const u32* blk = cls_pack + pi.round_off[0];
#pragma unroll
    for (u32 pp = 0; pp < 2; pp++) {
      const u32 e1 = tid + 256u * pp;
      const LN<9> w = NF ? pack_get<FT, 2>(blk, 1u << (S - 1), canon ? 1u : 0u, e1 >> LBT) : pack_get<FT, 2>(blk, SH::period2, canon ? 1u : 0u, e1);
      const LN<9> x = DIRECT ? xin[pp] : planes_get<FT>(lds, T, SWZ(e1));
      if (pp == 0) mem_phase(false);
      const bool cvs = NF && canon && SH::NR4 <= 1;
      if (zero_hi) {
        if constexpr (DIRECT) planes_put<FT>(lds, T, SWZ(e1), cvs ? ln::mul<FT>(x, k32) : x);
        planes_put<FT>(lds, T, SWZ(e1 + half), ln::mul<FT>(x, w));
      } else {
        const LN<9> y = DIRECT ? xin[pp + 2] : planes_get<FT>(lds, T, SWZ(e1 + half));
        LN<9> sum = ln::add(x, y);
        ln::normalize<FT>(sum);
        planes_put<FT>(lds, T, SWZ(e1), cvs ? ln::mul<FT>(sum, k32) : sum);
        planes_put<FT>(lds, T, SWZ(e1 + half), ln::mul<FT>(ln::sub(x, y), w));
      }
    }
    mem_phase(true);
    __syncthreads();
  }

  const u32 q = tid;
  if constexpr (NF && LAST) {
#pragma unroll
    for (int r = 0; r < 5; r++) {
      const int hb = 9 - 2 * r;
      const u32 D = 1u << (hb - 1);
      const u32 m = q >> (hb - 1);
      const u32 e0 = (m << (hb + 1)) | (q & (D - 1));
      const bool from_regs = DIRECT && r == 0;
      LN<9> x0 = from_regs ? xin[0] : planes_get<FT>(lds, T, SWZ(e0));
      const LN<9> x1 = from_regs ? xin[1] : planes_get<FT>(lds, T, SWZ(e0 + D));
      const LN<9> x2 = from_regs ? xin[2] : planes_get<FT>(lds, T, SWZ(e0 + 2 * D)), x3 = from_regs ? xin[3] : planes_get<FT>(lds, T, SWZ(e0 + 3 * D));
      LN<9> p1, p2, p3;
      if (r < 2) {
        const u32 sb = r == 0 ? 0u : (u32)__builtin_amdgcn_readfirstlane(tid >> 6);
        const u32* wu = cls_pack + pi.u_off + ((u32)r * 4 + sb) * (3 * U_SLOT<FT>);
        mem_phase(false);
        if (!from_regs) ln::clamp_apply<FT>(x0, ln::clamp_row<FT>(nqp, ln::clamp_q<FT>(x0.v[8])));
        p2 = ln::mul_u<FT>(x2, wu + U_SLOT<FT>);
        p1 = ln::mul_u<FT>(x1, wu);
        p3 = ln::mul_u<FT>(x3, wu + 2 * U_SLOT<FT>);
      } else {
        const u32* blk = cls_pack + pi.round_off[r];
        const LN<9> w1 = pack_get<FT, 3>(blk, coset_sets(r), 0, m), w2 = pack_get<FT, 3>(blk, coset_sets(r), 1, m);
        const LN<9> w3 = pack_get<FT, 3>(blk, coset_sets(r), 2, m);
        mem_phase(false);
        ln::clamp_apply<FT>(x0, ln::clamp_row<FT>(nqp, ln::clamp_q<FT>(x0.v[8])));
        p2 = ln::mul<FT>(x2, w2);
        p1 = ln::mul<FT>(x1, w1);
        p3 = ln::mul<FT>(x3, w3);
      }
      const LN<9> s02 = ln::add(x0, p2), d02 = ln::sub(x0, p2), s13 = ln::add(p1, p3);
      LN<9> y0 = ln::add(s02, s13), y1 = ln::sub(s02, s13);
      ln::normalize<FT>(y0);
      const LN<9> t = ln::mul_u<FT>(ln::sub(p1, p3), a.wq_w);
      LN<9> y2 = ln::add(d02, t), y3 = ln::sub(d02, t);
      if (r == 0 || r == 4) { ln::normalize<FT>(y1); ln::normalize<FT>(y2); ln::normalize<FT>(y3); }
      mem_phase(true);
      if (r < 4) {
        planes_put<FT>(lds, T, SWZ(e0), y0);
        planes_put<FT>(lds, T, SWZ(e0 + D), y1);
        planes_put<FT>(lds, T, SWZ(e0 + 2 * D), y2);
        planes_put<FT>(lds, T, SWZ(e0 + 3 * D), y3);
        __syncthreads();
      } else {
        u32* dstq = a.dst + row * a.dst_stride * NL + (size_t)((tile << S) | e0) * NL;
        LN<9> cc[4] = {y0, y1, y2, y3};
#pragma unroll
        for (int c = 0; c < 4; c++) {
          LN<9> x = cc[c];
          ln::clamp_apply<FT>(x, ln::clamp_row<FT>(nqp, ln::clamp_q<FT>(x.v[8])));
          u32 w[8];
          ln::to_packed<FT>(w, x.v);
          Fe<NL> v;
#pragma unroll
          for (int i = 0; i < 8; i++) v.v[i] = w[i];
          if (__any((int)(x.v[8] >= FT::limb(8)))) v = fe_reduce_once<8>(w);
          fe_store<NL>(dstq + (size_t)c * NL, v);
        }
      }
    }
    return;
  }
#pragma unroll
  for (int r = 0; r < SH::NR4; r++) {
    const int u = SH::U0 + 2 * r, hb = S - u - 1;
    const bool last_two = LAST && (r == SH::NR4 - 1);
    const bool triv = NF && FIRST && (r == SH::NR4 - 1);
    const u32 lp = q & ((1u << LBT) - 1), j = q >> LBT;
    const u32 i0 = ((j >> (hb - 1)) << (hb + 1)) | (j & ((1u << (hb - 1)) - 1));
    const u32 e0 = (i0 << LBT) | lp;
    constexpr u32 one = 1u;
    const u32 dq = one << (hb - 1 + LBT);
    const u32 period = NF ? one << (hb - 1) : one << (hb - 1 + LBT);
    const u32 jl = NF ? j & (period - 1) : q & (period - 1);
    const u32* blk = cls_pack + pi.round_off[SH::U0 + r];
    if (triv) {
      const bool fr = DIRECT && SH::U0 == 0 && r == 0;
      const LN<9> x0 = fr ? xin[0] : planes_get<FT>(lds, T, SWZ(e0)), x1 = fr ? xin[1] : planes_get<FT>(lds, T, SWZ(e0 + dq));
      const LN<9> x2 = fr ? xin[2] : planes_get<FT>(lds, T, SWZ(e0 + 2 * dq)), x3 = fr ? xin[3] : planes_get<FT>(lds, T, SWZ(e0 + 3 * dq));
      mem_phase(false);
      const LN<9> b0 = ln::add(x0, x2), b1 = ln::add(x1, x3);
      LN<9> c0 = ln::add(b0, b1), c1 = ln::sub(b0, b1);
      const LN<9> b2 = ln::sub(x0, x2);
      const LN<9> t = ln::mul_u<FT>(ln::sub(x1, x3), a.wq_w);
      LN<9> c2 = ln::add(b2, t), c3 = ln::sub(b2, t);
      ln::normalize<FT>(c1); ln::normalize<FT>(c2); ln::normalize<FT>(c3);
      if (RC < 0 && SH::U0 == 0 && canon) {
        ln::normalize<FT>(c0);
        c0 = ln::mul<FT>(c0, k32); c1 = ln::mul<FT>(c1, k32); c2 = ln::mul<FT>(c2, k32); c3 = ln::mul<FT>(c3, k32);
      } else if (fr) {
        ln::normalize<FT>(c0);
      } else {
        ln::clamp_apply<FT>(c0, ln::clamp_row<FT>(nqp, ln::clamp_q<FT>(c0.v[8])));
      }
      planes_put<FT>(lds, T, SWZ(e0), c0);
      planes_put<FT>(lds, T, SWZ(e0 + dq), c1);
      planes_put<FT>(lds, T, SWZ(e0 + 2 * dq), c2);
      planes_put<FT>(lds, T, SWZ(e0 + 3 * dq), c3);
      mem_phase(true);
      __syncthreads();
      continue;
    }
    if constexpr (RU >= 0) {
      if (r >= RU && !last_two) {
        const u32 wv = __builtin_amdgcn_readfirstlane(tid >> 6);
        const u32 qu = NF ? (((((tid & 63u) >> LBT) << 2) | wv) << LBT) | (tid & ((1u << LBT) - 1)) : ((tid & 63u) << 2) | wv;
        const u32 lpu = qu & ((1u << LBT) - 1), ju = qu >> LBT;
        const u32 iu = ((ju >> (hb - 1)) << (hb + 1)) | (ju & ((1u << (hb - 1)) - 1));
        const u32 eu = (iu << LBT) | lpu;
        const u32* wu = cls_pack + pi.u_off + ((r - RU) * 4 + wv) * (3 * U_SLOT<FT>);
        const LN<9> x0 = planes_get<FT>(lds, T, SWZ(eu)), x1 = planes_get<FT>(lds, T, SWZ(eu + dq));
        const LN<9> x2 = planes_get<FT>(lds, T, SWZ(eu + 2 * dq)), x3 = planes_get<FT>(lds, T, SWZ(eu + 3 * dq));
        mem_phase(false);
        const LN<9> b0 = ln::add(x0, x2), b1 = ln::add(x1, x3);
        LN<9> c0 = ln::add(b0, b1);
        ln::clamp_apply<FT>(c0, ln::clamp_row<FT>(nqp, ln::clamp_q<FT>(c0.v[8])));
        planes_put<FT>(lds, T, SWZ(eu), c0);
        LN<9> d1 = ln::sub(b0, b1);
        ln::normalize<FT>(d1);
        planes_put<FT>(lds, T, SWZ(eu + dq), ln::mul_u<FT>(d1, wu + 2 * U_SLOT<FT>));
        const LN<9> b2 = ln::mul_u<FT>(ln::sub(x0, x2), wu);
        const LN<9> b3 = ln::mul_u<FT>(ln::sub(x1, x3), wu + U_SLOT<FT>);
        LN<9> c2 = ln::add(b2, b3);
        if constexpr (NF) ln::clamp_apply<FT>(c2, ln::clamp_row<FT>(nqp, ln::clamp_q<FT>(c2.v[8])));
        else ln::normalize<FT>(c2);
        planes_put<FT>(lds, T, SWZ(eu + 2 * dq), c2);
        planes_put<FT>(lds, T, SWZ(eu + 3 * dq), ln::mul_u<FT>(ln::sub(b2, b3), wu + 2 * U_SLOT<FT>));
        mem_phase(true);
        __syncthreads();
        continue;
      }
    }
    if (u == 0 && zero_hi) {
      const u32 vb = canon ? 3u : 0u;
      const LN<9> w0 = pack_get<FT, 6>(blk, period, vb + 0, jl), w3 = pack_get<FT, 6>(blk, period, vb + 1, jl), w2 = pack_get<FT, 6>(blk, period, vb + 2, jl);
      mem_phase(false);
      const bool cv0 = NF && canon && r == RC;
      if (a.n_valid <= (1ull << (k - 2))) {
        const LN<9> x0 = DIRECT ? xin[0] : planes_get<FT>(lds, T, SWZ(e0));
        if constexpr (DIRECT) planes_put<FT>(lds, T, SWZ(e0), cv0 ? ln::mul<FT>(x0, k32) : x0);
        planes_put<FT>(lds, T, SWZ(e0 + dq), ln::mul<FT>(x0, w2));
        planes_put<FT>(lds, T, SWZ(e0 + 2 * dq), ln::mul<FT>(x0, w0));
        planes_put<FT>(lds, T, SWZ(e0 + 3 * dq), ln::mul<FT>(x0, w3));
      } else {
        const LN<9> x0 = DIRECT ? xin[0] : planes_get<FT>(lds, T, SWZ(e0)), x1 = DIRECT ? xin[1] : planes_get<FT>(lds, T, SWZ(e0 + dq));
        LN<9> c0 = ln::add(x0, x1);
        ln::normalize<FT>(c0);
        planes_put<FT>(lds, T, SWZ(e0), cv0 ? ln::mul<FT>(c0, k32) : c0);
        planes_put<FT>(lds, T, SWZ(e0 + dq), ln::mul<FT>(ln::sub(x0, x1), w2));
        const LN<9> t = ln::mul_u<FT>(x1, a.wq_w);
        planes_put<FT>(lds, T, SWZ(e0 + 2 * dq), ln::mul<FT>(ln::add(x0, t), w0));
        planes_put<FT>(lds, T, SWZ(e0 + 3 * dq), ln::mul<FT>(ln::sub(x0, t), w3));
      }
      mem_phase(true);
      __syncthreads();
      continue;
    }
    const bool from_regs = DIRECT && SH::U0 == 0 && r == 0;
    const LN<9> x0 = from_regs ? xin[0] : planes_get<FT>(lds, T, SWZ(e0)), x1 = from_regs ? xin[1] : planes_get<FT>(lds, T, SWZ(e0 + dq));
    const LN<9> x2 = from_regs ? xin[2] : planes_get<FT>(lds, T, SWZ(e0 + 2 * dq)), x3 = from_regs ? xin[3] : planes_get<FT>(lds, T, SWZ(e0 + 3 * dq));
    mem_phase(false);
    const LN<9> b0 = ln::add(x0, x2), b1 = ln::add(x1, x3);
    LN<9> c0 = ln::add(b0, b1);
    if (last_two) {
      ln::normalize<FT>(c0);
      LN<9> c1 = ln::sub(b0, b1);
      const LN<9> b2 = ln::sub(x0, x2);
      const LN<9> b3 = ln::mul_u<FT>(ln::sub(x1, x3), a.wq_w);
      LN<9> c2 = ln::add(b2, b3);
      LN<9> c3 = ln::sub(b2, b3);
      ln::normalize<FT>(c1); ln::normalize<FT>(c2); ln::normalize<FT>(c3);
      mem_phase(true);
      u32* dstq = a.dst + row * a.dst_stride * NL + (size_t)((tile << S) | e0) * NL;
      LN<9> cc[4] = {c0, c1, c2, c3};
#pragma unroll
      for (int c = 0; c < 4; c++) {
        LN<9> x = cc[c];
        ln::clamp_apply<FT>(x, ln::clamp_row<FT>(nqp, ln::clamp_q<FT>(x.v[8])));
        u32 w[8];
        ln::to_packed<FT>(w, x.v);
        Fe<NL> v;
#pragma unroll
        for (int i = 0; i < 8; i++) v.v[i] = w[i];
        if (__any((int)(x.v[8] >= FT::limb(8)))) v = fe_reduce_once<8>(w);
        fe_store<NL>(dstq + (size_t)c * NL, v);
      }
      return;
    } else {
      if (from_regs) ln::normalize<FT>(c0);
      else ln::clamp_apply<FT>(c0, ln::clamp_row<FT>(nqp, ln::clamp_q<FT>(c0.v[8])));
      planes_put<FT>(lds, T, SWZ(e0), c0);
      const bool blk0c = NF ? canon && q < dq : canon && blk0_tile && q < period && (RU < 0 || r < RU);
      if constexpr (NF ? RC >= 0 : RU >= 1) {
        if (r == (NF ? RC : RU - 1) && blk0c) {
          planes_put<FT>(lds, T, SWZ(e0), ln::mul<FT>(c0, k32));
        }
      }
      const u32 vb = blk0c ? 3u : 0u;
      const LN<9> w0 = pack_get<FT, 6>(blk, period, vb + 0, jl), w3 = pack_get<FT, 6>(blk, period, vb + 1, jl);
      const LN<9> w2 = pack_get<FT, 6>(blk, period, vb + 2, jl);
      const LN<9> d1 = ln::sub(b0, b1);
      planes_put<FT>(lds, T, SWZ(e0 + dq), ln::mul<FT>(d1, w2));
      const LN<9> t = ln::mul_u<FT>(ln::sub(x1, x3), a.wq_w);
      const LN<9> e2 = ln::sub(x0, x2);
      planes_put<FT>(lds, T, SWZ(e0 + 2 * dq), ln::mul<FT>(ln::add(e2, t), w0));
      planes_put<FT>(lds, T, SWZ(e0 + 3 * dq), ln::mul<FT>(ln::sub(e2, t), w3));
    }
    mem_phase(true);
    __syncthreads();
  }

  if constexpr (FIRST && MID) {
    u32* mrow = a.mid + (row << k) * 9;
#pragma unroll
    for (u32 e = tid; e < T; e += 256) {
      const u32 e2 = (tile << LTJ) | (e & ((1u << LBT) - 1));
      u32* t = mrow + (size_t)(e >> LBT) * (9 * T);
      const LN<9> x = planes_get<FT>(lds, T, SWZ(e));
      *reinterpret_cast<uint4*>(t + (size_t)e2 * 4) = make_uint4(x.v[0], x.v[1], x.v[2], x.v[3]);
      *reinterpret_cast<uint4*>(t + (size_t)(T + e2) * 4) = make_uint4(x.v[4], x.v[5], x.v[6], x.v[7]);
      t[(size_t)8 * T + e2] = x.v[8];
    }
    return;
  }
  if constexpr (FIRST) {
  u32* dst = a.dst + row * a.dst_stride * NL;
#pragma unroll
  for (u32 e = tid; e < T; e += 256) {
    const u32 g = gindex(e);
    LN<9> x = planes_get<FT>(lds, T, SWZ(e));
    ln::clamp_apply<FT>(x, ln::clamp_row<FT>(nqp, ln::clamp_q<FT>(x.v[8])));
    u32 w[8];
    ln::to_packed<FT>(w, x.v);
    Fe<NL> v;
#pragma unroll
    for (int i = 0; i < 8; i++) v.v[i] = w[i];
    fe_store<NL>(dst + (size_t)g * NL, v);
  }
  }
}

template <int S, int LTJ, bool FIRST, bool MID, bool NF>
hipError_t launch_tm(const NttPassArgs& a, const u32* pack, const NttPackInfo& pi, hipStream_t st) {
  constexpr int LT = S + LTJ;
  const u64 tiles = ((u64)1 << (a.log_n - LT)) * a.n_rows;
  const size_t lds_bytes = (((size_t)1 << LT) * 9 + 64 * LnField<FT255>::STRIDE) * 4;
  hipError_t e = hipFuncSetAttribute(reinterpret_cast<const void*>(&ntt_pass_l9s_kernel<S, LTJ, FIRST, MID, NF>),
                                     hipFuncAttributeMaxDynamicSharedMemorySize, (int)lds_bytes);
  if (e != hipSuccess) return e;
  hipLaunchKernelGGL((ntt_pass_l9s_kernel<S, LTJ, FIRST, MID, NF>), dim3((unsigned)tiles), dim3(256), lds_bytes, st, a, pack, pi);
  return hipGetLastError();
}
template <int S, int LTJ, bool FIRST>
hipError_t launch_t(const NttPassArgs& a, const u32* pack, const NttPackInfo& pi, hipStream_t st) {
  if (a.form) return a.mid ? launch_tm<S, LTJ, FIRST, true, true>(a, pack, pi, st) : launch_tm<S, LTJ, FIRST, false, true>(a, pack, pi, st);
  return a.mid ? launch_tm<S, LTJ, FIRST, true, false>(a, pack, pi, st) : launch_tm<S, LTJ, FIRST, false, false>(a, pack, pi, st);
}

}

bool ntt_l9s3_supported(uint32_t log_n) { return log_n >= 21 && log_n <= 26; }

bool ntt_l9s_supported(uint32_t log_n, uint32_t n_passes, int log_tile) { return n_passes == 2 && log_tile == 10 && log_n >= 11 && log_n <= 20; }

#define L9S_FIRST_CASES(X) X(1) X(2) X(3) X(4) X(5) X(6) X(7) X(8) X(9) X(10)

hipError_t launch_ntt_pass_l9s(const NttPassArgs& a, bool first, const uint32_t* pack, const NttPackInfo& pi, hipStream_t st) {
  if (!first) {
    if (a.s != 10 || a.log_tj != 0 || a.t0 + a.s != a.log_n) return hipErrorInvalidValue;
    if (a.mont_prefix) return hipErrorInvalidValue;
    return launch_t<10, 0, false>(a, pack, pi, st);
  }
  if (a.t0 != 0 || a.s + a.log_tj != 10 || (a.s + 10 != a.log_n && a.s + 20 != a.log_n)) return hipErrorInvalidValue;
  if (a.form && a.s + 10 != a.log_n) return hipErrorInvalidValue;
  if (a.tile_group && ((1u << (a.log_n - 10)) >> a.tile_group) < 8) return hipErrorInvalidValue;
  switch (a.s) {
#define X(SV) case SV: return launch_t<SV, 10 - SV, true>(a, pack, pi, st);
    L9S_FIRST_CASES(X)
#undef X
  }
  return hipErrorInvalidValue;
}

}
```

### lcpc_amd/csrc/ntt_lns.hip

```cpp
#include "kernels.h"
#include "ntt_ln_dev.h"

namespace lcpc {

namespace {

template <class FT> LCPC_DEV LN<FT::N> mul_i(const LN<FT::N>& x, const NttPassArgs& a) {
  if constexpr (ln::has_mul_u<FT>) return ln::mul_u<FT>(x, a.wq_w);
  else return ln::mul<FT>(x, tab_entry<FT>(a.roots29, 1u << (a.log_n - 2)));
}

constexpr u32 TILE = 1024;

template <class FT, int S, int LTJ, bool FIRST>
__global__ void __launch_bounds__(256, FT::WAVES) ntt_pass_lns_kernel(NttPassArgs a, const u32* __restrict__ pack, NttPackInfo pi) {
  constexpr int N = FT::N, NL = FT::NL, LBT = LTJ;
  constexpr bool LAST = !FIRST;
  static_assert(S + LTJ == 10, "1024-element tiles: one radix-4 quad (two radix-2 pairs) per thread and round");
  static_assert(FIRST || (LTJ == 0 && S % 2 == 0), "the last pass works on contiguous tiles and ends with the trivial stages k-2, k-1");
  using SH = Shape<S, LBT>;
  using E = LN<N>;
  constexpr u32 T = TILE;
  constexpr int RU = ln::has_mul_u<FT> ? SH::RU : -1;
  auto SWZ = [](u32 e) -> u32 { if constexpr (RU >= 0) return e ^ ((e >> 4) & 15u); else return e; };
  extern __shared__ __attribute__((aligned(16))) u32 lds[];
  u32* nqp = lds + (size_t)T * N;
  const u32 k = a.log_n;
  const u32 tiles_per_row = 1u << (k - 10);
  u64 row;
  u32 tile;
  if (FIRST && a.tile_group) {
    const u32 lg = a.tile_group;
    const u32 xcd = blockIdx.x & 7u;
    const u64 qq = blockIdx.x >> 3;
    const u32 sub = (u32)qq & ((1u << lg) - 1);
    const u64 q2 = qq >> lg;
    tile = (((u32)(q2 / a.n_rows) * 8u + xcd) << lg) | sub;
    row = q2 % a.n_rows;
  } else if (tiles_per_row >= 8) {
    const u32 xcd = blockIdx.x & 7u;
    const u64 qq = blockIdx.x >> 3;
    tile = (u32)(qq / a.n_rows) * 8u + xcd;
    row = qq % a.n_rows;
  } else {
    row = blockIdx.x / tiles_per_row;
    tile = blockIdx.x % tiles_per_row;
  }
  const u32 tid = threadIdx.x;
  mem_phase(true);
  const u32 lb = FIRST ? k - S : 0u;
  auto gindex = [&](u32 e) -> u32 {
    if constexpr (FIRST) return ((e >> LBT) << lb) | (tile << LTJ) | (e & ((1u << LBT) - 1));
    else return (tile << S) | e;
  };
  for (u32 i = tid; i < 64 * FT::STRIDE; i += 256) nqp[i] = 0u - a.qp29[i];
  const u32* src = a.src + row * a.src_stride * NL;
  constexpr bool DOUT = N <= 5;
  E xin[4];
#pragma unroll
  for (u32 it = 0; it < 4; it++) {
    const u32 e = tid + 256u * it;
    const u32 g = gindex(e);
    Fe<NL> v;
    if constexpr (FIRST) {
      v = (g < a.n_valid && row * a.src_stride + g < a.n_src_total) ? fe_load<NL>(src + (size_t)g * NL) : fe_zero<NL>();
      if (a.copy_dst != nullptr && g < a.n_valid) fe_store<NL>(a.copy_dst + (row * a.src_stride + g) * NL, v);
    } else {
      v = fe_load<NL>(src + (size_t)g * NL);
    }
    xin[it] = ln::from_packed<FT>(v);
  }
  const u32* cls_pack = pack + (size_t)(FIRST ? tile : 0u) * pi.class_words;
  const bool canon = a.roots29c != nullptr && ((u32)row & a.canon_row_mask) == 0;
  const bool blk0_tile = (FIRST || tile == 0) && a.blk0_gone == 0;
  const bool zero_hi = FIRST && a.n_valid <= (1ull << (k - 1));

  if constexpr (SH::U0 == 1) {
    constexpr u32 half = 1u << (S - 1 + LBT);
    const u32* blk = cls_pack + pi.round_off[0];
#pragma unroll
    for (u32 pp = 0; pp < 2; pp++) {
      const u32 e1 = tid + 256u * pp;
      const E w = pack_get<FT, 2>(blk, SH::period2, canon ? 1u : 0u, e1);
      const E x = xin[pp];
      if (pp == 0) mem_phase(false);
      if (zero_hi) {
        planes_put<FT>(lds, T, SWZ(e1), x);
        planes_put<FT>(lds, T, SWZ(e1 + half), ln::mul<FT>(x, w));
      } else {
        const E y = xin[pp + 2];
        E sum = ln::add(x, y);
        ln::normalize<FT>(sum);
        planes_put<FT>(lds, T, SWZ(e1), sum);
        planes_put<FT>(lds, T, SWZ(e1 + half), ln::mul<FT>(ln::sub(x, y), w));
      }
    }
    mem_phase(true);
    __syncthreads();
  }

  const u32 q = tid;
#pragma unroll
  for (int r = 0; r < SH::NR4; r++) {
    const int u = SH::U0 + 2 * r, hb = S - u - 1;
    const bool last_two = LAST && (r == SH::NR4 - 1);
    const u32 lp = q & ((1u << LBT) - 1), j = q >> LBT;
    const u32 i0 = ((j >> (hb - 1)) << (hb + 1)) | (j & ((1u << (hb - 1)) - 1));
    const u32 e0 = (i0 << LBT) | lp;
    constexpr u32 one = 1u;
    const u32 dq = one << (hb - 1 + LBT);
    const u32 period = one << (hb - 1 + LBT);
    const u32 jl = q & (period - 1);
    const u32* blk = cls_pack + pi.round_off[SH::U0 + r];
    if constexpr (RU >= 0) {
      if (r >= RU && !last_two) {
        const u32 wv = __builtin_amdgcn_readfirstlane(tid >> 6);
        const u32 qu = ((tid & 63u) << 2) | wv;
        const u32 lpu = qu & ((1u << LBT) - 1), ju = qu >> LBT;
        const u32 iu = ((ju >> (hb - 1)) << (hb + 1)) | (ju & ((1u << (hb - 1)) - 1));
        const u32 eu = (iu << LBT) | lpu;
        const u32* wu = cls_pack + pi.u_off + ((r - RU) * 4 + wv) * (3 * U_SLOT<FT>);
        const E x0 = planes_get<FT>(lds, T, SWZ(eu)), x1 = planes_get<FT>(lds, T, SWZ(eu + dq));
        const E x2 = planes_get<FT>(lds, T, SWZ(eu + 2 * dq)), x3 = planes_get<FT>(lds, T, SWZ(eu + 3 * dq));
        mem_phase(false);
        const E b0 = ln::add(x0, x2), b1 = ln::add(x1, x3);
        E c0 = ln::add(b0, b1);
        ln::clamp_apply<FT>(c0, ln::clamp_row<FT>(nqp, ln::clamp_q<FT>(c0.v[N - 1])));
        planes_put<FT>(lds, T, SWZ(eu), c0);
        E d1 = ln::sub(b0, b1);
        ln::normalize<FT>(d1);
        planes_put<FT>(lds, T, SWZ(eu + dq), ln::mul_u<FT>(d1, wu + 2 * U_SLOT<FT>));
        const E b2 = ln::mul_u<FT>(ln::sub(x0, x2), wu);
        const E b3 = ln::mul_u<FT>(ln::sub(x1, x3), wu + U_SLOT<FT>);
        E c2 = ln::add(b2, b3);
        ln::normalize<FT>(c2);
        planes_put<FT>(lds, T, SWZ(eu + 2 * dq), c2);
        planes_put<FT>(lds, T, SWZ(eu + 3 * dq), ln::mul_u<FT>(ln::sub(b2, b3), wu + 2 * U_SLOT<FT>));
        mem_phase(true);
        __syncthreads();
        continue;
      }
    }
    if (u == 0 && zero_hi) {
      const u32 vb = canon ? 3u : 0u;
      const E w0 = pack_get<FT, 6>(blk, period, vb + 0, jl), w2 = pack_get<FT, 6>(blk, period, vb + 2, jl);
      const E w3 = pack_get<FT, 6>(blk, period, vb + 1, jl);
      mem_phase(false);
      if (a.n_valid <= (1ull << (k - 2))) {
        const E x0 = xin[0];
        planes_put<FT>(lds, T, SWZ(e0), x0);
        planes_put<FT>(lds, T, SWZ(e0 + dq), ln::mul<FT>(x0, w2));
        planes_put<FT>(lds, T, SWZ(e0 + 2 * dq), ln::mul<FT>(x0, w0));
        planes_put<FT>(lds, T, SWZ(e0 + 3 * dq), ln::mul<FT>(x0, w3));
      } else {
        const E x0 = xin[0], x1 = xin[1];
        E c0 = ln::add(x0, x1);
        ln::normalize<FT>(c0);
        planes_put<FT>(lds, T, SWZ(e0), c0);
        planes_put<FT>(lds, T, SWZ(e0 + dq), ln::mul<FT>(ln::sub(x0, x1), w2));
        const E t = mul_i<FT>(x1, a);
        planes_put<FT>(lds, T, SWZ(e0 + 2 * dq), ln::mul<FT>(ln::add(x0, t), w0));
        planes_put<FT>(lds, T, SWZ(e0 + 3 * dq), ln::mul<FT>(ln::sub(x0, t), w3));
      }
      mem_phase(true);
      __syncthreads();
      continue;
    }
    const bool from_regs = SH::U0 == 0 && r == 0;
    const E x0 = from_regs ? xin[0] : planes_get<FT>(lds, T, SWZ(e0)), x1 = from_regs ? xin[1] : planes_get<FT>(lds, T, SWZ(e0 + dq));
    const E x2 = from_regs ? xin[2] : planes_get<FT>(lds, T, SWZ(e0 + 2 * dq)), x3 = from_regs ? xin[3] : planes_get<FT>(lds, T, SWZ(e0 + 3 * dq));
    mem_phase(false);
    const E b0 = ln::add(x0, x2), b1 = ln::add(x1, x3);
    E c0 = ln::add(b0, b1);
    if (last_two || from_regs) ln::normalize<FT>(c0);
    else ln::clamp_apply<FT>(c0, ln::clamp_row<FT>(nqp, ln::clamp_q<FT>(c0.v[N - 1])));
    if (!(last_two && DOUT)) planes_put<FT>(lds, T, SWZ(e0), c0);
    if (last_two) {
      E c1 = ln::sub(b0, b1);
      const E b2 = ln::sub(x0, x2);
      const E b3 = mul_i<FT>(ln::sub(x1, x3), a);
      E c2 = ln::add(b2, b3);
      E c3 = ln::sub(b2, b3);
      ln::normalize<FT>(c1); ln::normalize<FT>(c2); ln::normalize<FT>(c3);
      if constexpr (!DOUT) {
        planes_put<FT>(lds, T, SWZ(e0 + dq), c1);
        planes_put<FT>(lds, T, SWZ(e0 + 2 * dq), c2);
        planes_put<FT>(lds, T, SWZ(e0 + 3 * dq), c3);
      } else {
      mem_phase(true);
      u32* dstq = a.dst + row * a.dst_stride * NL + (size_t)((tile << S) | e0) * NL;
      E cc[4] = {c0, c1, c2, c3};
#pragma unroll
      for (int c = 0; c < 4; c++) {
        E x = cc[c];
        ln::clamp_apply<FT>(x, ln::clamp_row<FT>(nqp, ln::clamp_q<FT>(x.v[N - 1])));
        u32 w[NL];
        ln::to_packed<FT>(w, x.v);
        Fe<NL> v;
        if (__any((int)(x.v[N - 1] >= FT::limb(N - 1)))) v = fe_reduce_once<NL>(w, 0u);
        else {
#pragma unroll
          for (int i = 0; i < NL; i++) v.v[i] = w[i];
        }
        if (canon && tile == 0 && e0 + (u32)c < a.mont_prefix) v = fe_canon<NL>(v);
        fe_store<NL>(dstq + (size_t)c * NL, v);
      }
      return;
      }
    } else {
      const bool blk0c = canon && blk0_tile && q < period && (RU < 0 || r < RU);
      if constexpr (RU >= 1) {
        if (r == RU - 1 && blk0c) {
          E kc;
#pragma unroll
          for (int i = 0; i < N; i++) kc.v[i] = i == 0 ? (1u << (N * FT::W - 32 * NL)) : 0u;
          planes_put<FT>(lds, T, SWZ(e0), ln::mul<FT>(c0, kc));
        }
      }
      const u32 vb = blk0c ? 3u : 0u;
      const E w2 = pack_get<FT, 6>(blk, period, vb + 2, jl);
      planes_put<FT>(lds, T, SWZ(e0 + dq), ln::mul<FT>(ln::sub(b0, b1), w2));
      const E t = mul_i<FT>(ln::sub(x1, x3), a);
      const E e2 = ln::sub(x0, x2);
      const E w0 = pack_get<FT, 6>(blk, period, vb + 0, jl), w3 = pack_get<FT, 6>(blk, period, vb + 1, jl);
      planes_put<FT>(lds, T, SWZ(e0 + 2 * dq), ln::mul<FT>(ln::add(e2, t), w0));
      planes_put<FT>(lds, T, SWZ(e0 + 3 * dq), ln::mul<FT>(ln::sub(e2, t), w3));
    }
    mem_phase(true);
    __syncthreads();
  }

  if constexpr (FIRST || N > 5) {
  u32* dst = a.dst + row * a.dst_stride * NL;
#pragma unroll
  for (u32 e = tid; e < T; e += 256) {
    const u32 g = gindex(e);
    E x = planes_get<FT>(lds, T, SWZ(e));
    ln::clamp_apply<FT>(x, ln::clamp_row<FT>(nqp, ln::clamp_q<FT>(x.v[N - 1])));
    u32 w[NL];
    ln::to_packed<FT>(w, x.v);
    Fe<NL> v;
#pragma unroll
    for (int i = 0; i < NL; i++) v.v[i] = w[i];
    if constexpr (LAST) {
      if (__any((int)(x.v[N - 1] >= FT::limb(N - 1)))) v = fe_reduce_once<NL>(w, 0u);
      if (canon && tile == 0 && g < a.mont_prefix) v = fe_canon<NL>(v);
    }
    fe_store<NL>(dst + (size_t)g * NL, v);
  }
  }
}

template <class FT> LCPC_DEV LN<FT::N> tab_entry_neg(const u32* tab, u32 ix, u32 half_n) {
  LN<FT::N> m = tab_entry<FT>(tab, ix & (half_n - 1));
  if (ix >= half_n) {
    int32_t br = 0;
#pragma unroll
    for (int z = 0; z < FT::N; z++) {
      const int32_t d = (int32_t)FT::limb(z) - (int32_t)m.v[z] - br;
      br = d < 0 ? 1 : 0;
      m.v[z] = z + 1 < FT::N ? (u32)d & ((1u << FT::W) - 1) : (u32)d;
    }
  }
  return m;
}
template <class FT, int S, int LBT>
__global__ void __launch_bounds__(256) ntt_lns_pack_kernel(NttPassArgs a, NttPackInfo pi, u32 n_classes, bool first, u32* pack) {
  using SH = Shape<S, LBT>;
  constexpr u32 n_slots = SH::U0 + SH::NR4;
  constexpr u32 PMAX = 1u << (S - 1 + LBT);
  const u32 k = a.log_n, t0 = a.t0;
  const u32 lb = first ? k - S : 0u;
  const u64 total = (u64)n_classes * n_slots * PMAX;
  for (u64 id = (u64)blockIdx.x * 256 + threadIdx.x; id < total; id += (u64)gridDim.x * 256) {
    const u32 jl = (u32)(id % PMAX), slot = (u32)((id / PMAX) % n_slots), cls = (u32)(id / PMAX / n_slots);
    u32* blk = pack + (size_t)cls * pi.class_words + pi.round_off[slot];
    const u32 lo = first ? (cls << LBT) : 0u;
    if (SH::U0 == 1 && slot == 0) {
      const u32 lp = jl & ((1u << LBT) - 1), i = jl >> LBT;
      const u32 g1 = (i << lb) | lo | lp;
      const u32 gm = (1u << (k - t0 - 1)) - 1;
      pack_put<FT, 2>(blk, SH::period2, 0, jl, tab_entry<FT>(a.roots29, (g1 & gm) << t0));
      pack_put<FT, 2>(blk, SH::period2, 1, jl, tab_entry<FT>(a.roots29c, (g1 & gm) << t0));
      continue;
    }
    const u32 r = slot - SH::U0, u = SH::U0 + 2 * r, hb = S - u - 1, period = 1u << (hb - 1 + LBT);
    const u32 t = t0 + u;
    if (jl >= period || t + 2 == k) continue;
    const u32 gm0 = (1u << (k - t - 1)) - 1;
    const u32 lp = jl & ((1u << LBT) - 1), j = jl >> LBT;
    const u32 i0 = ((j >> (hb - 1)) << (hb + 1)) | (j & ((1u << (hb - 1)) - 1));
    const u32 g0 = (i0 << lb) | lo | lp;
    const u32 ex = (g0 & gm0) << t, half_n = 1u << (k - 1);
    const u32 idx[3] = {ex, 3 * ex, 2 * ex};
    for (u32 v = 0; v < 6; v++) pack_put<FT, 6>(blk, period, v, jl, tab_entry_neg<FT>(v < 3 ? a.roots29 : a.roots29c, idx[v % 3], half_n));
  }
}

template <class FT> LCPC_DEV void upack_write(const LN<FT::N>& w, u32* out) {
  constexpr int N = FT::N, W = FT::W;
  constexpr u32 M = (1u << W) - 1;
  for (u32 jj = 0; jj < (u32)N; jj++) {
    LN<N> sh;
#pragma unroll
    for (int z = 0; z < N; z++) sh.v[z] = (u32)z == jj ? 1u : 0u;
    LN<N> x = ln::mul<FT>(sh, w);
    LN<N> tt;
#pragma unroll
    for (int z = 0; z < N; z++) {
      const u32 hz = z + 1 < N ? ((FT::limb(z) >> 1) | ((FT::limb(z + 1) & 1u) << (W - 1))) : (FT::limb(z) >> 1);
      tt.v[z] = x.v[z] + hz;
    }
    ln::normalize<FT>(tt);
    if ((int32_t)tt.v[N - 1] < 0) {
#pragma unroll
      for (int z = 0; z < N; z++) x.v[z] += FT::limb(z);
      ln::normalize<FT>(x);
    }
#pragma unroll
    for (int kk = 0; kk < N; kk++) out[N * kk + jj] = kk + 1 < N ? (x.v[kk] & M) : x.v[kk];
  }
  for (u32 z = N * N; z < U_SLOT<FT>; z++) out[z] = 0;
}
template <class FT, int S, int LBT>
__global__ void __launch_bounds__(64) ntt_lns_upack_kernel(NttPassArgs a, NttPackInfo pi, u32 n_classes, bool first, u32* pack) {
  using SH = Shape<S, LBT>;
  const u32 k = a.log_n, t0 = a.t0;
  const u32 lb = first ? k - S : 0u;
  const u32 id = blockIdx.x * 64 + threadIdx.x;
  if (id >= n_classes * SH::NRU * 12) return;
  const u32 cls = id / (SH::NRU * 12), ru = (id / 12) % SH::NRU, jl0 = (id % 12) / 3, v = id % 3;
  const u32 r = SH::RU + ru;
  const u32 u = SH::U0 + 2 * r, hb = S - u - 1;
  const u32 t = t0 + u;
  if (t + 2 == k) return;
  const u32 jl = jl0 & (SH::period4(r) - 1);
  const u32 lo = first ? (cls << LBT) : 0u;
  const u32 gm0 = (1u << (k - t - 1)) - 1, gm1 = gm0 >> 1;
  const u32 lp = jl & ((1u << LBT) - 1), j = jl >> LBT;
  const u32 i0 = ((j >> (hb - 1)) << (hb + 1)) | (j & ((1u << (hb - 1)) - 1));
  const u32 g0 = (i0 << lb) | lo | lp;
  const u32 g1 = g0 + (1u << (hb - 1 + lb));
  const u32 idx = v == 0 ? (g0 & gm0) << t : (v == 1 ? (g1 & gm0) << t : (g0 & gm1) << (t + 1));
  const LN<FT::N> w = tab_entry<FT>(a.roots29, idx);
  upack_write<FT>(w, pack + (size_t)cls * pi.class_words + pi.u_off + ((ru * 4 + jl0) * 3 + v) * U_SLOT<FT>);
}

using F255 = LnField<FT255>;
__global__ void __launch_bounds__(64) l9s_pure_upack_kernel(NttPassArgs a, NttPackInfo pi, u32 u, u32* pack) {
  const u32 id = threadIdx.x;
  if (id >= 12) return;
  const u32 jl0 = id / 3, v = id % 3;
  const u32 k = a.log_n, lb = k - a.s, hb = a.s - u - 1;
  const u32 gm0 = (1u << (k - u - 1)) - 1, gm1 = gm0 >> 1;
  const u32 g0 = jl0 << lb, g1 = g0 + (1u << (hb - 1 + lb));
  const u32 idx = v == 0 ? (g0 & gm0) << u : (v == 1 ? (g1 & gm0) << u : (g0 & gm1) << (u + 1));
  upack_write<F255>(tab_entry<F255>(a.roots29, idx), pack + pi.u_off + (jl0 * 3 + v) * U_SLOT<F255>);
}
LCPC_DEV u32 coset_exp(u32 k, u32 cls, u32 r, u32 m) {
  const u32 S = k - 10;
  const u32 k1 = __brev(cls) >> (32 - S);
  const u32 rm = r ? __brev(m) >> (32 - 2 * r) : 0u;
  return (k1 + (rm << S)) << (8 - 2 * r);
}
__global__ void __launch_bounds__(256) l9s_coset_pack_kernel(NttPassArgs a, NttPackInfo pi, u32 n_classes, u32* pack) {
  const u32 k = a.log_n, half_n = 1u << (k - 1);
  const u64 total = (u64)n_classes * 336;
  for (u64 id = (u64)blockIdx.x * 256 + threadIdx.x; id < total; id += (u64)gridDim.x * 256) {
    const u32 cls = (u32)(id / 336), x = (u32)(id % 336);
    const u32 r = x < 16 ? 2u : (x < 80 ? 3u : 4u), m = x < 16 ? x : (x < 80 ? x - 16 : x - 80);
    const u32 E = coset_exp(k, cls, r, m);
    u32* blk = pack + (size_t)cls * pi.class_words + pi.round_off[r];
    for (u32 v = 0; v < 3; v++) pack_put<F255, 3>(blk, coset_sets(r), v, m, tab_entry_neg<F255>(a.roots29, (v + 1) * E, half_n));
  }
}
__global__ void __launch_bounds__(64) l9s_coset_upack_kernel(NttPassArgs a, NttPackInfo pi, u32 n_classes, u32* pack) {
  const u32 k = a.log_n, half_n = 1u << (k - 1);
  const u32 id = blockIdx.x * 64 + threadIdx.x;
  if (id >= n_classes * 15) return;
  const u32 cls = id / 15, x = id % 15;
  const u32 r = x < 3 ? 0u : 1u, m = x < 3 ? 0u : (x - 3) / 3, v = x % 3;
  const u32 E = coset_exp(k, cls, r, m);
  upack_write<F255>(tab_entry_neg<F255>(a.roots29, (v + 1) * E, half_n), pack + (size_t)cls * pi.class_words + pi.u_off + ((r * 4 + m) * 3 + v) * U_SLOT<F255>);
}

template <class FT, int S, int LBT> NttPackInfo pack_info_t() {
  using SH = Shape<S, LBT>;
  NttPackInfo pi{};
  u32 off = 0, slot = 0;
  if (SH::U0) { pi.round_off[slot++] = off; off += 2 * SH::period2 * FT::N; off = (off + 3) & ~3u; }
  for (int r = 0; r < SH::NR4; r++) { pi.round_off[slot++] = off; off += 6 * SH::period4(r) * FT::N; off = (off + 3) & ~3u; }
  if (ln::has_mul_u<FT> && SH::RU >= 0) { off = (off + U_ALIGN<FT> - 1) & ~(U_ALIGN<FT> - 1); pi.u_off = off; off += SH::NRU * 4 * 3 * U_SLOT<FT>; }
  pi.class_words = off;
  return pi;
}

template <class FT, int S, int LTJ, bool FIRST>
hipError_t launch_t(const NttPassArgs& a, const u32* pack, const NttPackInfo& pi, hipStream_t st) {
  const u64 tiles = ((u64)1 << (a.log_n - 10)) * a.n_rows;
  const size_t lds_bytes = ((size_t)TILE * FT::N + 64 * FT::STRIDE) * 4;
  hipLaunchKernelGGL((ntt_pass_lns_kernel<FT, S, LTJ, FIRST>), dim3((unsigned)tiles), dim3(256), lds_bytes, st, a, pack, pi);
  return hipGetLastError();
}

template <class FT>
__global__ void __launch_bounds__(256) roots_ln_kernel(const u32* roots, u64 n, const u32* rprime, u32* out) {
  const u64 i = (u64)blockIdx.x * 256 + threadIdx.x;
  if (i >= n) return;
  const Fe<FT::NL> c = fe_load<FT::NL>(rprime);
  const Fe<FT::NL> t = fe_mul<FT::NL>(fe_load<FT::NL>(roots + i * FT::NL), c);
  const LN<FT::N> l = ln::from_packed<FT>(t);
#pragma unroll
  for (int k = 0; k < FT::STRIDE; k++) out[i * FT::STRIDE + k] = k < FT::N ? l.v[k] : 0u;
}

#define LNS_FIRST_CASES(X) X(1) X(2) X(3) X(4) X(5) X(6) X(7) X(8) X(9) X(10)

NttPackInfo form_pack_info(uint32_t s, bool first) {
  NttPackInfo pi{};
  u32 off = 0;
  if (first) {
    const u32 u0 = s & 1, nr4 = s / 2;
    u32 slot = 0;
    if (u0) { pi.round_off[slot++] = off; off += 2 * (1u << (s - 1)) * 9; off = (off + 3) & ~3u; }
    for (u32 r = 0; r < nr4; r++) { pi.round_off[slot++] = off; off += 6 * (1u << (s - u0 - 2 * r - 2)) * 9; off = (off + 3) & ~3u; }
    if (nr4 >= 3) { pi.u_off = off; off += 4 * 3 * U_SLOT<F255>; }
  } else {
    for (u32 r = 2; r < 5; r++) { pi.round_off[r] = off; off += 3 * coset_sets(r) * 9; }
    pi.u_off = off;
    off += 2 * 4 * 3 * U_SLOT<F255>;
  }
  pi.class_words = off;
  return pi;
}

template <class FT> NttPackInfo pack_info_f(uint32_t s, bool first) {
  if (!first) return pack_info_t<FT, 10, 0>();
  switch (s) {
#define X(SV) case SV: return pack_info_t<FT, SV, 10 - SV>();
    LNS_FIRST_CASES(X)
#undef X
  }
  return NttPackInfo{};
}
template <class FT> hipError_t launch_pack_f(const NttPassArgs& a, bool first, const NttPackInfo& pi, uint32_t n_classes, uint32_t* pack, hipStream_t st) {
  const unsigned ugrid = (n_classes * 2 * 12 + 63) / 64;
  if (!first) {
    hipLaunchKernelGGL((ntt_lns_pack_kernel<FT, 10, 0>), dim3(64), dim3(256), 0, st, a, pi, n_classes, false, pack);
    if constexpr (ln::has_mul_u<FT>) hipLaunchKernelGGL((ntt_lns_upack_kernel<FT, 10, 0>), dim3(ugrid), dim3(64), 0, st, a, pi, n_classes, false, pack);
    return hipGetLastError();
  }
  switch (a.s) {
#define X(SV) case SV: hipLaunchKernelGGL((ntt_lns_pack_kernel<FT, SV, 10 - SV>), dim3(2048), dim3(256), 0, st, a, pi, n_classes, true, pack); break;
    LNS_FIRST_CASES(X)
#undef X
    default: return hipErrorInvalidValue;
  }
  if constexpr (ln::has_mul_u<FT>) {
    if (a.s == 8) hipLaunchKernelGGL((ntt_lns_upack_kernel<FT, 8, 2>), dim3(ugrid), dim3(64), 0, st, a, pi, n_classes, true, pack);
    if (a.s == 9) hipLaunchKernelGGL((ntt_lns_upack_kernel<FT, 9, 1>), dim3(ugrid), dim3(64), 0, st, a, pi, n_classes, true, pack);
    if (a.s == 10) hipLaunchKernelGGL((ntt_lns_upack_kernel<FT, 10, 0>), dim3(ugrid), dim3(64), 0, st, a, pi, n_classes, true, pack);
  }
  return hipGetLastError();
}
template <class FT> hipError_t launch_pass_f(const NttPassArgs& a, bool first, const uint32_t* pack, const NttPackInfo& pi, hipStream_t st) {
  if (!first) {
    if (a.s != 10 || a.log_tj != 0 || a.t0 + a.s != a.log_n) return hipErrorInvalidValue;
    return launch_t<FT, 10, 0, false>(a, pack, pi, st);
  }
  if (a.t0 != 0 || a.s + a.log_tj != 10 || (a.s + 10 != a.log_n && a.s + 20 != a.log_n)) return hipErrorInvalidValue;
  switch (a.s) {
#define X(SV) case SV: return launch_t<FT, SV, 10 - SV, true>(a, pack, pi, st);
    LNS_FIRST_CASES(X)
#undef X
  }
  return hipErrorInvalidValue;
}

}

#define LNS_DISPATCH(nl, EXPR)                         \
  switch (nl) {                                        \
    case 2: { using FT = LnField<FT63>; EXPR; }        \
    case 4: { using FT = LnField<FT127>; EXPR; }       \
    case 6: { using FT = LnField<FT191>; EXPR; }       \
    case 8: { using FT = LnField<FT255>; EXPR; }       \
    default: break;                                    \
  }

NttPackInfo ntt_l9s_form_pack_info(uint32_t s, bool first) { return form_pack_info(s, first); }
hipError_t launch_ntt_l9s_form_pack(const NttPassArgs& a, bool first, const NttPackInfo& pi, uint32_t n_classes, uint32_t* pack, hipStream_t st) {
  if (a.log_n < 11 || a.log_n > 20 || a.s != (first ? a.log_n - 10 : 10u)) return hipErrorInvalidValue;
  if (!first) {
    hipLaunchKernelGGL(l9s_coset_pack_kernel, dim3(n_classes >= 1024 ? 1344u : (n_classes * 336 + 255) / 256), dim3(256), 0, st, a, pi, n_classes, pack);
    hipLaunchKernelGGL(l9s_coset_upack_kernel, dim3((n_classes * 15 + 63) / 64), dim3(64), 0, st, a, pi, n_classes, pack);
    return hipGetLastError();
  }
  if (n_classes != 1) return hipErrorInvalidValue;
  switch (a.s) {
#define X(SV) case SV: hipLaunchKernelGGL((ntt_lns_pack_kernel<F255, SV, 0>), dim3(4), dim3(256), 0, st, a, pi, 1u, true, pack); break;
    LNS_FIRST_CASES(X)
#undef X
  }
  const u32 u0 = a.s & 1, nr4 = a.s / 2;
  if (nr4 >= 3) hipLaunchKernelGGL(l9s_pure_upack_kernel, dim3(1), dim3(64), 0, st, a, pi, u0 + 2 * (nr4 - 2), pack);
  return hipGetLastError();
}
bool ntt_lns_supported(int nl, uint32_t log_n) { return (nl == 2 || nl == 4 || nl == 6) && log_n >= 11 && log_n <= 20u; }
bool ntt_lns3_supported(int nl, uint32_t log_n) { return (nl == 2 || nl == 4 || nl == 6) && log_n >= 21 && log_n <= 26; }
__global__ void __launch_bounds__(256) lns_subtable_kernel(const u32* tab, u32 shift, u64 n, u32 words, u32* sub) {
  for (u64 id = (u64)blockIdx.x * 256 + threadIdx.x; id < n * words; id += (u64)gridDim.x * 256) {
    const u64 i = id / words, w = id % words;
    sub[i * words + w] = tab[(i << shift) * words + w];
  }
}
hipError_t launch_ntt_lns_subtable(int nl, const uint32_t* tab, uint32_t shift, uint64_t n, uint32_t* sub, hipStream_t st) {
  hipLaunchKernelGGL(lns_subtable_kernel, dim3(2048), dim3(256), 0, st, tab, shift, n, (u32)ntt_lns_stride(nl), sub);
  return hipGetLastError();
}
int ntt_lns_limbs(int nl) { LNS_DISPATCH(nl, return FT::N) return 0; }
int ntt_lns_limb_bits(int nl) { LNS_DISPATCH(nl, return FT::W) return 0; }
int ntt_lns_stride(int nl) { LNS_DISPATCH(nl, return FT::STRIDE) return 0; }

NttPackInfo ntt_lns_pack_info(int nl, uint32_t s, bool first) {
  LNS_DISPATCH(nl, return pack_info_f<FT>(s, first))
  return NttPackInfo{};
}
hipError_t launch_ntt_lns_roots(int nl, const uint32_t* roots, uint64_t n, const uint32_t* rprime, uint32_t* out, hipStream_t st) {
  const dim3 grid((unsigned)((n + 255) / 256));
  LNS_DISPATCH(nl, hipLaunchKernelGGL((roots_ln_kernel<FT>), grid, dim3(256), 0, st, roots, n, rprime, out); return hipGetLastError())
  return hipErrorInvalidValue;
}
hipError_t launch_ntt_lns_pack(int nl, const NttPassArgs& a, bool first, const NttPackInfo& pi, uint32_t n_classes, uint32_t* pack, hipStream_t st) {
  LNS_DISPATCH(nl, return launch_pack_f<FT>(a, first, pi, n_classes, pack, st))
  return hipErrorInvalidValue;
}
hipError_t launch_ntt_pass_lns(int nl, const NttPassArgs& a, bool first, const uint32_t* pack, const NttPackInfo& pi, hipStream_t st) {
  if (a.tile_group && (!first || ((1u << (a.log_n - 10)) >> a.tile_group) < 8)) return hipErrorInvalidValue;
  switch (nl) {
    case 2: return launch_pass_f<LnField<FT63>>(a, first, pack, pi, st);
    case 4: return launch_pass_f<LnField<FT127>>(a, first, pack, pi, st);
    case 6: return launch_pass_f<LnField<FT191>>(a, first, pack, pi, st);
  }
  return hipErrorInvalidValue;
}

}
```

Baseline: 7.319 billion.

## Add two-table split twiddle multiply for Ft255 pure/coset NTT passes

Introduces a two-table twiddle multiply for the 255-bit field. Each twiddle is stored as two precomputed constants (w·2^145 and w·2^290 mod p), so the product can be formed as a low-half and high-half dot product with a shorter Montgomery-style reduction (5 reduction digits instead of a full one), emitted as generated inline asm. The pack tables double in size for the affected rounds, and a runtime switch plus default heuristic picks it per pass when s0 fits. The aim is to cut the ALU cost of each butterfly multiply, paid for with more twiddle loads and memory, and with wider intermediate ranges.

Result: faster. 7.603 billion, median of 6 (+3.9%).

```diff
diff --git a/lcpc_amd/csrc/ctx.cpp b/lcpc_amd/csrc/ctx.cpp
--- a/lcpc_amd/csrc/ctx.cpp
+++ b/lcpc_amd/csrc/ctx.cpp
@@ -163,6 +163,7 @@
   return std::min(std::min(lg, 6u), tiles_log - 3);
 }
 
+static bool ntt_mul_split_default(unsigned s0, bool first) { return first ? s0 == 8 : s0 >= 6; }
 static int build_limb_plan(lcpc_ctx* c, unsigned n_pass) {
   std::vector<uint32_t**> made;
   std::vector<NttStep> plan(n_pass);
@@ -216,7 +217,8 @@
       const bool nf = c->L == 4 && n_pass == 2 && (c->sw_ntt_form == 1 || (c->sw_ntt_form < 0 && s0 >= 6));
       p.a.form = nf ? 1u : 0u;
       if (nf && last) p.blk0_gone = 1u;
-      p.pack_info = nf ? ntt_l9s_form_pack_info(p.a.s, p.first) : ntt_lns_pack_info(c->NL, p.a.s, p.first);
+      const bool m2 = nf && ntt_l9s_mul2_supported(p.a.s, p.first) && (c->sw_ntt_mul == 1 || c->sw_ntt_mul == (p.first ? 2 : 3) || (c->sw_ntt_mul < 0 && ntt_mul_split_default(s0, p.first)));
+      p.pack_info = nf ? ntt_l9s_form_pack_info(p.a.s, p.first, m2) : ntt_lns_pack_info(c->NL, p.a.s, p.first);
       const uint32_t n_classes = p.first != nf ? 1u << (p.a.log_n - 10) : 1u;
 #ifdef LCPC_TEST_HOOKS
       if (n_pass == 3 && i == 0 && c->sw_test_fail_3pass) return LCPC_ERR_NOMEM;
@@ -228,6 +230,10 @@
       else HIPCHK(c, launch_ntt_lns_pack(c->NL, pa, p.first, p.pack_info, n_classes, p.pack, nullptr));
     }
     HIPCHK(c, hipDeviceSynchronize());
+    if (c->sw_debug_timing)
+      for (unsigned i = 0; i < n_pass; i++)
+        fprintf(stderr, "lcpc: ntt plan 2^%u pass %u/%u: %s s=%u form=%u mul2=%u\n", k, i + 1, n_pass, plan[i].kernel == NttStep::K1S ? "K1s" : "K1n",
+                plan[i].a.s, plan[i].a.form, plan[i].pack_info.mul2);
     return 0;
   }();
   if (rc == 0) {
@@ -554,6 +560,7 @@
   if (c->prm.sdig_code == 0) c->prm.sdig_code = 3;
   c->sw_ntt_general = getenv("LCPC_NTT_GENERAL") != nullptr;
   if (const char* ev = getenv("LCPC_NTT_FORM")) c->sw_ntt_form = !strcmp(ev, "dif") ? 0 : (!strcmp(ev, "coset") ? 1 : -1);
+  if (const char* ev = getenv("LCPC_NTT_MUL")) c->sw_ntt_mul = !strcmp(ev, "mont") ? 0 : (!strcmp(ev, "split") ? 1 : (!strcmp(ev, "split-pure") ? 2 : (!strcmp(ev, "split-coset") ? 3 : -1)));
   if (const char* ev = getenv("LCPC_NTT_MID_MAX_MB")) c->sw_ntt_mid_max_mb = (int64_t)strtoull(ev, nullptr, 10);
   if (const char* ev = getenv("LCPC_HOST_STAGE")) c->sw_host_stage = (int32_t)strtol(ev, nullptr, 10);
   c->sw_debug_timing = getenv("LCPC_DEBUG_TIMING") != nullptr;
diff --git a/lcpc_amd/csrc/field_ln.h b/lcpc_amd/csrc/field_ln.h
--- a/lcpc_amd/csrc/field_ln.h
+++ b/lcpc_amd/csrc/field_ln.h
@@ -126,6 +126,30 @@
   else r29_mul1s(a.v, w.v, r.v);
   return r;
 }
+template <class FT> LCPC_DEV LN<FT::N> mul2(const LN<FT::N>& a, const LN<FT::N>& b0, const LN<FT::N>& b1) {
+  static_assert(FT::FID == FT255, "the two-table multiply exists for Ft255 only");
+  LN<FT::N> r = b1;
+  r29_mul2s(a.v, b0.v, r.v);
+  return r;
+}
+template <class FT> LCPC_DEV void mul2_pair(const LN<FT::N>& e, LN<FT::N>& b0, LN<FT::N>& b1) {
+  static_assert(FT::FID == FT255, "the two-table multiply exists for Ft255 only");
+#pragma unroll
+  for (int t = 0; t < 2; t++) {
+    LN<FT::N> kk;
+#pragma unroll
+    for (int z = 0; z < FT::N; z++) kk.v[z] = t ? R29_MUL2_KB[z] : R29_MUL2_KA[z];
+    LN<FT::N> x = mul<FT>(kk, e);
+    for (int it = 0; it < 2; it++) {
+      if ((int32_t)x.v[FT::N - 1] < 0) {
+#pragma unroll
+        for (int z = 0; z < FT::N; z++) x.v[z] += FT::limb(z);
+        normalize<FT>(x);
+      }
+    }
+    (t ? b1 : b0) = x;
+  }
+}
 template <class FT> constexpr bool has_mul_u = FT::N >= 5;
 template <class FT> LCPC_DEV LN<FT::N> mul_u(const LN<FT::N>& a, const u32* wt) {
   static_assert(has_mul_u<FT>, "no shifted-multiples multiply for this field");
diff --git a/lcpc_amd/csrc/gen/gen_r29_asm.py b/lcpc_amd/csrc/gen/gen_r29_asm.py
--- a/lcpc_amd/csrc/gen/gen_r29_asm.py
+++ b/lcpc_amd/csrc/gen/gen_r29_asm.py
@@ -101,6 +101,57 @@
 out.append("// One-statement multiplies; they clobber v[%d:%d], s[%d:%d], vcc.  The asserts tie the literals to LnField<FT255>." % (ACC, ACC + 1, PS, PS + N - 2))
 for j in range(1, N):
     out.append("static_assert(LnField<FT255>::limb(%d) == 0x%xu, \"gen_r29_asm.py modulus\");" % (j, (FT255_P >> (29 * j)) & ((1 << 29) - 1)))
-emit("r29_mul1s", "// signed form (ln::mul<LnField<FT255>>): x limbs two's complement, |x_k| < 2^30, |value| < 16p; b as above.\n"
-     "// r = x * b * 2^-261 in (-1.2p, 0.2p]: limbs 0..7 in [0, 2^29), top limb signed.", mul1(True))
-print("\n".join(out))
+
+
+ND2 = 5
+def mul2():
+    mad, shr = "v_mad_i64_i32", "v_ashrrev_i64"
+    ins = []
+    for j in range(1, N):
+        pj = (FT255_P >> (29 * j)) & ((1 << 29) - 1)
+        ins.append("s_mov_b32 s%d, 0x%x" % (PS + j - 1, (-pj) & 0xffffffff))
+    first = True
+    for k in range(N + ND2 - 1):
+        for i in range(ND2):
+            j = k - i
+            if 0 <= j < N:
+                ins.append("%s %s, vcc, %%[x%d], %%[a%d], %s" % (mad, acc, i, j, "0" if first else acc))
+                first = False
+        for i in range(N - ND2):
+            j = k - i
+            if 0 <= j < N:
+                ins.append("%s %s, vcc, %%[x%d], %%[r%d], %s" % (mad, acc, ND2 + i, j, acc))
+        for i in range(ND2):
+            j = k - i
+            if i < k and 1 <= j < N:
+                ins.append("%s %s, vcc, %%[m%d], s%d, %s" % (mad, acc, i, PS + j - 1, acc))
+        ins.append("v_and_b32 %%[%s], 0x1fffffff, %s" % ("m%d" % k if k < ND2 else "r%d" % (k - ND2), lo))
+        ins.append("%s %s, 29, %s" % (shr, acc, acc))
+    ins.append("v_mov_b32 %%[r%d], %s" % (N - 1, lo))
+    return ins
+
+
+def emit2(name, comment, ins):
+    out.append("")
+    out.append(comment)
+    out.append("LCPC_DEV void %s(const u32* x, const u32* a, u32* r) {" % name)
+    out.append("  u32 m0, m1, m2, m3, m4;")
+    out.append("  asm(")
+    for t in ins:
+        out.append('      "%s\\n\\t"' % t)
+    outs = ", ".join(['[r%d] "+v"(r[%d])' % (k, k) for k in range(N)] + ['[m%d] "=&v"(m%d)' % (k, k) for k in range(ND2)])
+    inps = ", ".join(['[x%d] "v"(x[%d])' % (i, i) for i in range(N)] + ['[a%d] "v"(a[%d])' % (j, j) for j in range(N)])
+    clob = ", ".join(['"vcc"', '"v%d"' % ACC, '"v%d"' % (ACC + 1)] + ['"s%d"' % (PS + j) for j in range(N - 1)])
+    out.append("      : %s\n      : %s\n      : %s);" % (outs, inps, clob))
+    out.append("}")
+
+
+if __name__ == "__main__":
+  emit("r29_mul1s", "// signed form (ln::mul<LnField<FT255>>): x limbs two's complement, |x_k| < 2^30, |value| < 16p; b as above.\n"
+       "// r = x * b * 2^-261 in (-1.2p, 0.2p]: limbs 0..7 in [0, 2^29), top limb signed.", mul1(True))
+  emit2("r29_mul2s", "// two-table form (ln::mul2<LnField<FT255>>): x limbs two's complement, |x_k| < 2^30; a = w c 2^145 mod p and, in r on entry,\n"
+        "// b = w c 2^290 mod p, both in [0, p).  r = (XL a + XH b) 2^-145 == x w c in (-3.01p, 2.01p): limbs 0..7 in [0, 2^29), top limb signed.", mul2())
+  for nm, e in (("R29_MUL2_KA", 145), ("R29_MUL2_KB", 290)):
+      v = pow(2, e, FT255_P)
+      out.append("constexpr u32 %s[9] = {%s};" % (nm, ", ".join("0x%xu" % ((v >> (29 * k)) & ((1 << 29) - 1)) for k in range(N))))
+  print("\n".join(out))
diff --git a/lcpc_amd/csrc/internal.h b/lcpc_amd/csrc/internal.h
--- a/lcpc_amd/csrc/internal.h
+++ b/lcpc_amd/csrc/internal.h
@@ -219,6 +219,7 @@
 struct lcpc_ctx {
   lcpc_params prm{};
   bool sw_ntt_general = false;
+  int sw_ntt_mul = -1;
   int sw_ntt_form = -1;
   int64_t sw_ntt_mid_max_mb = -1;
   bool sw_debug_timing = false;
diff --git a/lcpc_amd/csrc/kernels.h b/lcpc_amd/csrc/kernels.h
--- a/lcpc_amd/csrc/kernels.h
+++ b/lcpc_amd/csrc/kernels.h
@@ -31,11 +31,13 @@
   uint32_t round_off[8];
   uint32_t class_words;
   uint32_t u_off;
+  uint32_t mul2;
 };
 bool ntt_l9s_supported(uint32_t log_n, uint32_t n_passes, int log_tile);
 bool ntt_l9s3_supported(uint32_t log_n);
 hipError_t launch_ntt_pass_l9s(const NttPassArgs& a, bool first, const uint32_t* pack, const NttPackInfo& pi, hipStream_t st);
-NttPackInfo ntt_l9s_form_pack_info(uint32_t s, bool first);
+NttPackInfo ntt_l9s_form_pack_info(uint32_t s, bool first, bool mul2);
+constexpr bool ntt_l9s_mul2_supported(uint32_t s, bool first) { return !first ? s == 10 : (s >= 1 && s <= 10 && s != 2 && s != 7 && s != 9); }
 hipError_t launch_ntt_l9s_form_pack(const NttPassArgs& a, bool first, const NttPackInfo& pi, uint32_t n_classes, uint32_t* pack, hipStream_t st);
 
 bool ntt_lns_supported(int nl, uint32_t log_n);
diff --git a/lcpc_amd/csrc/ntt_l9s.hip b/lcpc_amd/csrc/ntt_l9s.hip
--- a/lcpc_amd/csrc/ntt_l9s.hip
+++ b/lcpc_amd/csrc/ntt_l9s.hip
@@ -5,13 +5,32 @@
 
 namespace {
 
-template <int S, int LTJ, bool FIRST, bool MID, bool NF>
+template <bool M2> struct Tw { LN<9> b0, b1; };
+template <> struct Tw<false> { LN<9> b0; };
+template <bool M2, u32 NV> LCPC_DEV Tw<M2> tw_get(const u32* blk, u32 period, u32 variant, u32 jl) {
+  using FT = LnField<FT255>;
+  Tw<M2> t;
+  if constexpr (M2) {
+    t.b0 = pack_get<FT, 2 * NV>(blk, period, variant, jl);
+    t.b1 = pack_get<FT, 2 * NV>(blk, period, NV + variant, jl);
+  } else {
+    t.b0 = pack_get<FT, NV>(blk, period, variant, jl);
+  }
+  return t;
+}
+template <bool M2> LCPC_DEV LN<9> tw_mul(const LN<9>& x, const Tw<M2>& w) {
+  if constexpr (M2) return ln::mul2<LnField<FT255>>(x, w.b0, w.b1);
+  else return ln::mul<LnField<FT255>>(x, w.b0);
+}
+
+template <int S, int LTJ, bool FIRST, bool MID, bool NF, bool M2>
 __global__ void __launch_bounds__(256, 4) ntt_pass_l9s_kernel(NttPassArgs a, const u32* __restrict__ pack, NttPackInfo pi) {
   using FT = LnField<FT255>;
   constexpr int NL = 8, LT = S + LTJ, LBT = LTJ;
   constexpr bool LAST = !FIRST;
   static_assert(LT == 10, "1024-element tiles: one radix-4 quad (two radix-2 pairs) per thread and round");
   static_assert(FIRST || (LTJ == 0 && S % 2 == 0), "the last pass works on contiguous tiles and ends with the trivial stages k-2, k-1");
+  static_assert(NF || !M2, "the two-table multiply serves the pure / coset form only");
   using SH = Shape<S, LBT>;
   using SP = PureShape<S>;
   constexpr int RU = NF ? (FIRST ? SP::RU : -1) : SH::RU;
@@ -105,19 +124,19 @@
 #pragma unroll
     for (u32 pp = 0; pp < 2; pp++) {
       const u32 e1 = tid + 256u * pp;
-      const LN<9> w = NF ? pack_get<FT, 2>(blk, 1u << (S - 1), canon ? 1u : 0u, e1 >> LBT) : pack_get<FT, 2>(blk, SH::period2, canon ? 1u : 0u, e1);
+      const Tw<M2> w = NF ? tw_get<M2, 2>(blk, 1u << (S - 1), canon ? 1u : 0u, e1 >> LBT) : tw_get<M2, 2>(blk, SH::period2, canon ? 1u : 0u, e1);
       const LN<9> x = DIRECT ? xin[pp] : planes_get<FT>(lds, T, SWZ(e1));
       if (pp == 0) mem_phase(false);
       const bool cvs = NF && canon && SH::NR4 <= 1;
       if (zero_hi) {
         if constexpr (DIRECT) planes_put<FT>(lds, T, SWZ(e1), cvs ? ln::mul<FT>(x, k32) : x);
-        planes_put<FT>(lds, T, SWZ(e1 + half), ln::mul<FT>(x, w));
+        planes_put<FT>(lds, T, SWZ(e1 + half), tw_mul<M2>(x, w));
       } else {
         const LN<9> y = DIRECT ? xin[pp + 2] : planes_get<FT>(lds, T, SWZ(e1 + half));
         LN<9> sum = ln::add(x, y);
         ln::normalize<FT>(sum);
         planes_put<FT>(lds, T, SWZ(e1), cvs ? ln::mul<FT>(sum, k32) : sum);
-        planes_put<FT>(lds, T, SWZ(e1 + half), ln::mul<FT>(ln::sub(x, y), w));
+        planes_put<FT>(lds, T, SWZ(e1 + half), tw_mul<M2>(ln::sub(x, y), w));
       }
     }
     mem_phase(true);
@@ -147,13 +166,13 @@
         p3 = ln::mul_u<FT>(x3, wu + 2 * U_SLOT<FT>);
       } else {
         const u32* blk = cls_pack + pi.round_off[r];
-        const LN<9> w1 = pack_get<FT, 3>(blk, coset_sets(r), 0, m), w2 = pack_get<FT, 3>(blk, coset_sets(r), 1, m);
-        const LN<9> w3 = pack_get<FT, 3>(blk, coset_sets(r), 2, m);
+        const Tw<M2> w1 = tw_get<M2, 3>(blk, coset_sets(r), 0, m), w2 = tw_get<M2, 3>(blk, coset_sets(r), 1, m);
+        const Tw<M2> w3 = tw_get<M2, 3>(blk, coset_sets(r), 2, m);
         mem_phase(false);
         ln::clamp_apply<FT>(x0, ln::clamp_row<FT>(nqp, ln::clamp_q<FT>(x0.v[8])));
-        p2 = ln::mul<FT>(x2, w2);
-        p1 = ln::mul<FT>(x1, w1);
-        p3 = ln::mul<FT>(x3, w3);
+        p2 = tw_mul<M2>(x2, w2);
+        p1 = tw_mul<M2>(x1, w1);
+        p3 = tw_mul<M2>(x3, w3);
       }
       const LN<9> s02 = ln::add(x0, p2), d02 = ln::sub(x0, p2), s13 = ln::add(p1, p3);
       LN<9> y0 = ln::add(s02, s13), y1 = ln::sub(s02, s13);
@@ -259,24 +278,24 @@
     }
     if (u == 0 && zero_hi) {
       const u32 vb = canon ? 3u : 0u;
-      const LN<9> w0 = pack_get<FT, 6>(blk, period, vb + 0, jl), w3 = pack_get<FT, 6>(blk, period, vb + 1, jl), w2 = pack_get<FT, 6>(blk, period, vb + 2, jl);
+      const Tw<M2> w0 = tw_get<M2, 6>(blk, period, vb + 0, jl), w3 = tw_get<M2, 6>(blk, period, vb + 1, jl), w2 = tw_get<M2, 6>(blk, period, vb + 2, jl);
       mem_phase(false);
       const bool cv0 = NF && canon && r == RC;
       if (a.n_valid <= (1ull << (k - 2))) {
         const LN<9> x0 = DIRECT ? xin[0] : planes_get<FT>(lds, T, SWZ(e0));
         if constexpr (DIRECT) planes_put<FT>(lds, T, SWZ(e0), cv0 ? ln::mul<FT>(x0, k32) : x0);
-        planes_put<FT>(lds, T, SWZ(e0 + dq), ln::mul<FT>(x0, w2));
-        planes_put<FT>(lds, T, SWZ(e0 + 2 * dq), ln::mul<FT>(x0, w0));
-        planes_put<FT>(lds, T, SWZ(e0 + 3 * dq), ln::mul<FT>(x0, w3));
+        planes_put<FT>(lds, T, SWZ(e0 + dq), tw_mul<M2>(x0, w2));
+        planes_put<FT>(lds, T, SWZ(e0 + 2 * dq), tw_mul<M2>(x0, w0));
+        planes_put<FT>(lds, T, SWZ(e0 + 3 * dq), tw_mul<M2>(x0, w3));
       } else {
         const LN<9> x0 = DIRECT ? xin[0] : planes_get<FT>(lds, T, SWZ(e0)), x1 = DIRECT ? xin[1] : planes_get<FT>(lds, T, SWZ(e0 + dq));
         LN<9> c0 = ln::add(x0, x1);
         ln::normalize<FT>(c0);
         planes_put<FT>(lds, T, SWZ(e0), cv0 ? ln::mul<FT>(c0, k32) : c0);
-        planes_put<FT>(lds, T, SWZ(e0 + dq), ln::mul<FT>(ln::sub(x0, x1), w2));
+        planes_put<FT>(lds, T, SWZ(e0 + dq), tw_mul<M2>(ln::sub(x0, x1), w2));
         const LN<9> t = ln::mul_u<FT>(x1, a.wq_w);
-        planes_put<FT>(lds, T, SWZ(e0 + 2 * dq), ln::mul<FT>(ln::add(x0, t), w0));
-        planes_put<FT>(lds, T, SWZ(e0 + 3 * dq), ln::mul<FT>(ln::sub(x0, t), w3));
+        planes_put<FT>(lds, T, SWZ(e0 + 2 * dq), tw_mul<M2>(ln::add(x0, t), w0));
+        planes_put<FT>(lds, T, SWZ(e0 + 3 * dq), tw_mul<M2>(ln::sub(x0, t), w3));
       }
       mem_phase(true);
       __syncthreads();
@@ -323,14 +342,26 @@
         }
       }
       const u32 vb = blk0c ? 3u : 0u;
-      const LN<9> w0 = pack_get<FT, 6>(blk, period, vb + 0, jl), w3 = pack_get<FT, 6>(blk, period, vb + 1, jl);
-      const LN<9> w2 = pack_get<FT, 6>(blk, period, vb + 2, jl);
+      if constexpr (M2) {
+        const Tw<M2> w2 = tw_get<M2, 6>(blk, period, vb + 2, jl), w0 = tw_get<M2, 6>(blk, period, vb + 0, jl);
+        const LN<9> d1 = ln::sub(b0, b1);
+        const LN<9> d13 = ln::sub(x1, x3), e2 = ln::sub(x0, x2);
+        planes_put<FT>(lds, T, SWZ(e0 + dq), tw_mul<M2>(d1, w2));
+        __builtin_amdgcn_sched_barrier(0);
+        const Tw<M2> w3 = tw_get<M2, 6>(blk, period, vb + 1, jl);
+        const LN<9> t = ln::mul_u<FT>(d13, a.wq_w);
+        planes_put<FT>(lds, T, SWZ(e0 + 2 * dq), tw_mul<M2>(ln::add(e2, t), w0));
+        planes_put<FT>(lds, T, SWZ(e0 + 3 * dq), tw_mul<M2>(ln::sub(e2, t), w3));
+      } else {
+      const Tw<M2> w0 = tw_get<M2, 6>(blk, period, vb + 0, jl), w3 = tw_get<M2, 6>(blk, period, vb + 1, jl);
+      const Tw<M2> w2 = tw_get<M2, 6>(blk, period, vb + 2, jl);
       const LN<9> d1 = ln::sub(b0, b1);
-      planes_put<FT>(lds, T, SWZ(e0 + dq), ln::mul<FT>(d1, w2));
+      planes_put<FT>(lds, T, SWZ(e0 + dq), tw_mul<M2>(d1, w2));
       const LN<9> t = ln::mul_u<FT>(ln::sub(x1, x3), a.wq_w);
       const LN<9> e2 = ln::sub(x0, x2);
-      planes_put<FT>(lds, T, SWZ(e0 + 2 * dq), ln::mul<FT>(ln::add(e2, t), w0));
-      planes_put<FT>(lds, T, SWZ(e0 + 3 * dq), ln::mul<FT>(ln::sub(e2, t), w3));
+      planes_put<FT>(lds, T, SWZ(e0 + 2 * dq), tw_mul<M2>(ln::add(e2, t), w0));
+      planes_put<FT>(lds, T, SWZ(e0 + 3 * dq), tw_mul<M2>(ln::sub(e2, t), w3));
+      }
     }
     mem_phase(true);
     __syncthreads();
@@ -366,21 +397,25 @@
   }
 }
 
-template <int S, int LTJ, bool FIRST, bool MID, bool NF>
+template <int S, int LTJ, bool FIRST, bool MID, bool NF, bool M2>
 hipError_t launch_tm(const NttPassArgs& a, const u32* pack, const NttPackInfo& pi, hipStream_t st) {
   constexpr int LT = S + LTJ;
   const u64 tiles = ((u64)1 << (a.log_n - LT)) * a.n_rows;
   const size_t lds_bytes = (((size_t)1 << LT) * 9 + 64 * LnField<FT255>::STRIDE) * 4;
-  hipError_t e = hipFuncSetAttribute(reinterpret_cast<const void*>(&ntt_pass_l9s_kernel<S, LTJ, FIRST, MID, NF>),
+  hipError_t e = hipFuncSetAttribute(reinterpret_cast<const void*>(&ntt_pass_l9s_kernel<S, LTJ, FIRST, MID, NF, M2>),
                                      hipFuncAttributeMaxDynamicSharedMemorySize, (int)lds_bytes);
   if (e != hipSuccess) return e;
-  hipLaunchKernelGGL((ntt_pass_l9s_kernel<S, LTJ, FIRST, MID, NF>), dim3((unsigned)tiles), dim3(256), lds_bytes, st, a, pack, pi);
+  hipLaunchKernelGGL((ntt_pass_l9s_kernel<S, LTJ, FIRST, MID, NF, M2>), dim3((unsigned)tiles), dim3(256), lds_bytes, st, a, pack, pi);
   return hipGetLastError();
 }
 template <int S, int LTJ, bool FIRST>
 hipError_t launch_t(const NttPassArgs& a, const u32* pack, const NttPackInfo& pi, hipStream_t st) {
-  if (a.form) return a.mid ? launch_tm<S, LTJ, FIRST, true, true>(a, pack, pi, st) : launch_tm<S, LTJ, FIRST, false, true>(a, pack, pi, st);
-  return a.mid ? launch_tm<S, LTJ, FIRST, true, false>(a, pack, pi, st) : launch_tm<S, LTJ, FIRST, false, false>(a, pack, pi, st);
+  if (pi.mul2) {
+    if constexpr (ntt_l9s_mul2_supported(S, FIRST)) { if (a.form) return a.mid ? launch_tm<S, LTJ, FIRST, true, true, true>(a, pack, pi, st) : launch_tm<S, LTJ, FIRST, false, true, true>(a, pack, pi, st); }
+    return hipErrorInvalidValue;
+  }
+  if (a.form) return a.mid ? launch_tm<S, LTJ, FIRST, true, true, false>(a, pack, pi, st) : launch_tm<S, LTJ, FIRST, false, true, false>(a, pack, pi, st);
+  return a.mid ? launch_tm<S, LTJ, FIRST, true, false, false>(a, pack, pi, st) : launch_tm<S, LTJ, FIRST, false, false, false>(a, pack, pi, st);
 }
 
 }
diff --git a/lcpc_amd/csrc/ntt_lns.hip b/lcpc_amd/csrc/ntt_lns.hip
--- a/lcpc_amd/csrc/ntt_lns.hip
+++ b/lcpc_amd/csrc/ntt_lns.hip
@@ -264,6 +264,18 @@
   }
   return m;
 }
+template <class FT, u32 NV> LCPC_DEV void pack_put_tw(u32* blk, u32 period, u32 variant, u32 jl, const LN<FT::N>& e, u32 mul2) {
+  if constexpr (FT::FID == FT255) {
+    if (mul2) {
+      LN<FT::N> b0, b1;
+      ln::mul2_pair<FT>(e, b0, b1);
+      pack_put<FT, 2 * NV>(blk, period, variant, jl, b0);
+      pack_put<FT, 2 * NV>(blk, period, NV + variant, jl, b1);
+      return;
+    }
+  }
+  pack_put<FT, NV>(blk, period, variant, jl, e);
+}
 template <class FT, int S, int LBT>
 __global__ void __launch_bounds__(256) ntt_lns_pack_kernel(NttPassArgs a, NttPackInfo pi, u32 n_classes, bool first, u32* pack) {
   using SH = Shape<S, LBT>;
@@ -280,8 +292,8 @@
       const u32 lp = jl & ((1u << LBT) - 1), i = jl >> LBT;
       const u32 g1 = (i << lb) | lo | lp;
       const u32 gm = (1u << (k - t0 - 1)) - 1;
-      pack_put<FT, 2>(blk, SH::period2, 0, jl, tab_entry<FT>(a.roots29, (g1 & gm) << t0));
-      pack_put<FT, 2>(blk, SH::period2, 1, jl, tab_entry<FT>(a.roots29c, (g1 & gm) << t0));
+      pack_put_tw<FT, 2>(blk, SH::period2, 0, jl, tab_entry<FT>(a.roots29, (g1 & gm) << t0), pi.mul2);
+      pack_put_tw<FT, 2>(blk, SH::period2, 1, jl, tab_entry<FT>(a.roots29c, (g1 & gm) << t0), pi.mul2);
       continue;
     }
     const u32 r = slot - SH::U0, u = SH::U0 + 2 * r, hb = S - u - 1, period = 1u << (hb - 1 + LBT);
@@ -293,7 +305,7 @@
     const u32 g0 = (i0 << lb) | lo | lp;
     const u32 ex = (g0 & gm0) << t, half_n = 1u << (k - 1);
     const u32 idx[3] = {ex, 3 * ex, 2 * ex};
-    for (u32 v = 0; v < 6; v++) pack_put<FT, 6>(blk, period, v, jl, tab_entry_neg<FT>(v < 3 ? a.roots29 : a.roots29c, idx[v % 3], half_n));
+    for (u32 v = 0; v < 6; v++) pack_put_tw<FT, 6>(blk, period, v, jl, tab_entry_neg<FT>(v < 3 ? a.roots29 : a.roots29c, idx[v % 3], half_n), pi.mul2);
   }
 }
 
@@ -371,7 +383,7 @@
     const u32 r = x < 16 ? 2u : (x < 80 ? 3u : 4u), m = x < 16 ? x : (x < 80 ? x - 16 : x - 80);
     const u32 E = coset_exp(k, cls, r, m);
     u32* blk = pack + (size_t)cls * pi.class_words + pi.round_off[r];
-    for (u32 v = 0; v < 3; v++) pack_put<F255, 3>(blk, coset_sets(r), v, m, tab_entry_neg<F255>(a.roots29, (v + 1) * E, half_n));
+    for (u32 v = 0; v < 3; v++) pack_put_tw<F255, 3>(blk, coset_sets(r), v, m, tab_entry_neg<F255>(a.roots29, (v + 1) * E, half_n), pi.mul2);
   }
 }
 __global__ void __launch_bounds__(64) l9s_coset_upack_kernel(NttPassArgs a, NttPackInfo pi, u32 n_classes, u32* pack) {
@@ -416,17 +428,19 @@
 
 #define LNS_FIRST_CASES(X) X(1) X(2) X(3) X(4) X(5) X(6) X(7) X(8) X(9) X(10)
 
-NttPackInfo form_pack_info(uint32_t s, bool first) {
+NttPackInfo form_pack_info(uint32_t s, bool first, bool mul2) {
   NttPackInfo pi{};
   u32 off = 0;
+  const u32 nb = mul2 ? 2u : 1u;
+  pi.mul2 = mul2 ? 1u : 0u;
   if (first) {
     const u32 u0 = s & 1, nr4 = s / 2;
     u32 slot = 0;
-    if (u0) { pi.round_off[slot++] = off; off += 2 * (1u << (s - 1)) * 9; off = (off + 3) & ~3u; }
-    for (u32 r = 0; r < nr4; r++) { pi.round_off[slot++] = off; off += 6 * (1u << (s - u0 - 2 * r - 2)) * 9; off = (off + 3) & ~3u; }
+    if (u0) { pi.round_off[slot++] = off; off += nb * 2 * (1u << (s - 1)) * 9; off = (off + 3) & ~3u; }
+    for (u32 r = 0; r < nr4; r++) { pi.round_off[slot++] = off; off += nb * 6 * (1u << (s - u0 - 2 * r - 2)) * 9; off = (off + 3) & ~3u; }
     if (nr4 >= 3) { pi.u_off = off; off += 4 * 3 * U_SLOT<F255>; }
   } else {
-    for (u32 r = 2; r < 5; r++) { pi.round_off[r] = off; off += 3 * coset_sets(r) * 9; }
+    for (u32 r = 2; r < 5; r++) { pi.round_off[r] = off; off += nb * 3 * coset_sets(r) * 9; }
     pi.u_off = off;
     off += 2 * 4 * 3 * U_SLOT<F255>;
   }
@@ -488,7 +502,7 @@
     default: break;                                    \
   }
 
-NttPackInfo ntt_l9s_form_pack_info(uint32_t s, bool first) { return form_pack_info(s, first); }
+NttPackInfo ntt_l9s_form_pack_info(uint32_t s, bool first, bool mul2) { return form_pack_info(s, first, mul2); }
 hipError_t launch_ntt_l9s_form_pack(const NttPassArgs& a, bool first, const NttPackInfo& pi, uint32_t n_classes, uint32_t* pack, hipStream_t st) {
   if (a.log_n < 11 || a.log_n > 20 || a.s != (first ? a.log_n - 10 : 10u)) return hipErrorInvalidValue;
   if (!first) {
```
